# MrGiovanni/R-Super

Hardware: AMD Instinct MI355X
Metric: CT voxels/sec/node (96³ patch, bs=2/GPU) (higher is better)
Workload: dtype bf16; 1 GPU; R-Super 3D UNet(base 32, 26 classes, BasicBlock/IN) full training step (fwd + masked BCE + Dice loss + bwd + clip + AdamW + EMA), 96^3 patches, batch 2/GPU (BASELINE.json configs[1]); global_batch=2, patch=96, parallelism=dp1, sanity_checks_form=device-side flags read one step late (train_ddp.StepGuard)

## Files before the change

include/rsuper_hip.h:

```cpp
#ifndef RSUPER_HIP_H
#define RSUPER_HIP_H
#include <stddef.h>
#include <stdint.h>
#ifdef __cplusplus
extern "C" {
#endif

#define RSUPER_F32 0
#define RSUPER_BF16 1
#define RSUPER_OK 0
#define RSUPER_ERR_ARG 1
#define RSUPER_ERR_LAUNCH 2
#define RSUPER_ERR_UNSUPPORTED 3
#define RSUPER_ERR_NO_DEVICE 4

const char* rsuper_version(void);
int rsuper_device_check(void);


size_t rsuper_conv3_packed_elems(int dtype, int ka, int kb, int n_cols, int bn);

int rsuper_conv3_pack_weights(int dtype, int mode, const float* wa, const float* wb, int ka, int kb, int na, int nb,
                              int bn, void* packed, void* stream);

int rsuper_conv3_pack_weights_batch(int dtype, int n, const int* host_desc, const float* const* host_wa, const float* const* host_wb,
                                    const size_t* host_out_elems, void* packed, void* stream);

int rsuper_conv3_tiles(int D, int H, int W);

int rsuper_conv3_variant(int v);
int rsuper_conv3_wgrad2_min_tiles(int t);

int rsuper_conv3_plan(int dtype, int epi, int N, int D, int H, int W, int Ca, int Cb, int n_cols, int src_flags, int bn, int* plan);

int rsuper_conv3_box_bn(int dtype, int N, int D, int H, int W, int n_cols);

int rsuper_conv3_kd_bn(int dtype, int epi, int N, int D, int H, int W, int n_cols, int src_flags);

int rsuper_conv3_set_workspace(void* ptr, size_t bytes);
size_t rsuper_conv3_workspace_bytes(void);

int rsuper_conv3_part_rows(int dtype, int epi, int N, int D, int H, int W, int n_cols, int bn, int src_flags);

int rsuper_conv3_igemm(int dtype, int epi,
                       const void* xa, int lda, int Ca, const float* mra,
                       const void* xb, int ldb, int Cb, const float* mrb,
                       const void* packed, int n_cols, int bn, int N, int D, int H, int W,
                       void* out, int ldo, const void* res, int ldr, float* part,
                       const void* exa, int elda, int eCa, const float* emra,
                       const void* exb, int eldb, int eCb, const float* emrb, void* stream);
int rsuper_conv3_igemm_split_out(int dtype, int epi,
                                 const void* xa, int lda, int Ca, const float* mra,
                                 const void* xb, int ldb, int Cb, const float* mrb,
                                 const void* packed, int n_cols, int bn, int N, int D, int H, int W,
                                 void* out, int ldo, const void* res, int ldr, float* part,
                                 const void* exa, int elda, int eCa, const float* emra,
                                 const void* exb, int eldb, int eCb, const float* emrb, int out_split, long long out_part, void* stream);
int rsuper_conv3_s2_part_rows(int dtype, int mode, int Ca, int Cb, int n_cols, int N, int FD, int FH, int FW);
int rsuper_conv3_igemm_s2(int dtype, int mode, const void* xa, int lda, int Ca, const float* mra,
                          const void* xb, int ldb, int Cb, const void* packed, int n_cols, int N, int FD, int FH, int FW,
                          void* out, int ldo, float* part, const void* exa, int elda, const float* emra, void* stream);

int rsuper_conv3_wgrad_plan(int dtype, int use_tr, int Ca, int Cb, int Ya, int Yb, int N, int D, int H, int W, int src_flags, int splits, int* plan);
int rsuper_conv3_wgrad_splits(int dtype, int Ca, int Cb, int Ya, int Yb, int N, int D, int H, int W);

int rsuper_conv3_wgrad(int dtype, int use_tr,
                       const void* xa, int lda, int Ca, const float* mra,
                       const void* xb, int ldb, int Cb, const float* mrb,
                       const void* ya, int ldya, int Ya, const void* yb, int ldyb, int Yb,
                       float* dwa, float* dwb, float* workspace, int N, int D, int H, int W, int splits, void* stream);

int rsuper_conv3_wgrad_partial(int dtype, int use_tr, const void* xa, int lda, int Ca, const float* mra,
                               const void* xb, int ldb, int Cb, const float* mrb,
                               const void* ya, int ldya, int Ya, const void* yb, int ldyb, int Yb,
                               float* workspace, int N, int D, int H, int W, int splits, void* stream);
int rsuper_conv3_wgrad_reduce(const float* workspace, int splits, int Cin, int Ya, int Yb, float* dwa, float* dwb, void* stream);
int rsuper_conv3_wgrad_reduce_batch(int n, const void* const* workspaces, const int* splits, const int* Cin, const int* Ya, const int* Yb,
                                    void* const* dwa, void* const* dwb, void* stream);
int rsuper_conv3_wgrad_reduce_batch_stats(int n, const void* const* workspaces, const int* splits, const int* Cin, const int* Ya, const int* Yb,
                                           void* const* dwa, void* const* dwb, int nstats, const void* const* parts, const int* sN, const int* snblk,
                                           const int* sC, const double* scnt, const int* smode, const int* ssplit, void* const* souts, float eps, void* stream);

int rsuper_conv3_wgrad_s2_splits(int dtype, int Ca, int Mtot, int N, int FD, int FH, int FW);
int rsuper_conv3_wgrad_s2(int dtype, const void* xa, int lda, int Ca, const float* mra,
                          const void* ya, int ldya, int Ya, const void* yb, int ldyb, int Yb,
                          float* dwa, float* dwb, float* workspace, int N, int FD, int FH, int FW, int splits, void* stream);

size_t rsuper_pointwise_packed_bytes(int dtype, int K, int N);
int rsuper_pointwise(int dtype, int mode, const float* x, int ldx, const float* w, const float* bias, const float* res, int ldr,
                     float* y, int ldy, long R, int K, int N, void* packed, void* stream);
int rsuper_pointwise_pack_batch(int dtype, const long long* table, int n, long total_items, void* arena, void* stream);
int rsuper_pointwise_wgrad_splits(long R, int N, int K);
int rsuper_pointwise_wgrad(int dtype, const float* dy, int ldy, const float* x, int ldx, long R, int N, int K, float* workspace, int splits,
                           float* dw, float* db, void* stream);

int rsuper_stats_finalize(const float* part, int N, int nblk, int C, double cnt, float eps, int mode, int split, float* out, void* stream);
int rsuper_glue_variant(int v);
int rsuper_in_bwd_finalize(int dtype, const void* g, int ldg, const void* x, int ldx, const float* mr, const float* gm,
                           const void* add1, int lda1, const void* add2, int lda2, void* out, int ldo,
                           int N, int vox, int C, void* stream);

int rsuper_maxpool2_fwd(int dtype, const void* x, int ldx, void* y, int ldy, float* part, int blocks,
                        int N, int D, int H, int W, int C, void* stream);
int rsuper_maxpool2_bwd(int dtype, const void* x, int ldx, const void* dy, int lddy, void* dx, int lddx,
                        int N, int D, int H, int W, int C, void* stream);
int rsuper_maxpool2_bwd_add(int dtype, const void* x, int ldx, const void* dy, int lddy, const void* add, int lda, void* dx, int lddx,
                            int N, int D, int H, int W, int C, void* stream);

int rsuper_subsample2_fwd(int dtype, const void* x, int ldx, void* y, int ldy, float* part, int blocks,
                          int N, int D, int H, int W, int C, void* stream);
int rsuper_subsample2_bwd(int dtype, const void* dy, int lddy, void* dx, int lddx, int N, int D, int H, int W, int C, void* stream);

int rsuper_upsample_fwd(int dtype, const void* x, int ldx, void* y, int ldy, float* part, int blocks,
                        int N, int ID, int IH, int IW, int OD, int OH, int OW, int C, void* stream);
int rsuper_upsample_bwd(int dtype, const void* dy, int lddy, void* dx, int lddx,
                        int N, int ID, int IH, int IW, int OD, int OH, int OW, int C, void* stream);

int rsuper_stem_fwd(int dtype, const float* x, const float* w, void* y, int ldy, float* part,
                    int N, int D, int H, int W, int C, void* stream);
int rsuper_stem_wgrad(int dtype, const float* x, const void* dy, int lddy, float* dw, int N, int D, int H, int W, int C, void* stream);

int rsuper_head_fwd(int dtype, const void* x, int ldx, const float* w, const float* b, float* logits, int N, int vox, int C, int K, void* stream);
int rsuper_head_bwd_data(int dtype, const float* dlogits, const float* w, void* dx, int lddx, int N, int vox, int C, int K, void* stream);
int rsuper_head_bwd_weight(int dtype, const void* x, int ldx, const float* dlogits, float* dw, float* db, int N, int vox, int C, int K, void* stream);
int rsuper_head_bwd(int dtype, const void* x, int ldx, const float* dlogits, const float* w, void* dx, int lddx, float* dw, float* db,
                    int N, int vox, int C, int K, void* stream);

int rsuper_plane_partials_fwd(const float* x, size_t xstride, const uint8_t* t, const uint8_t* k, const float* w1, const uint8_t* w2,
                              double* sums, int flags, int planes, size_t V, void* stream);
int rsuper_plane_partials_bwd(const float* x, size_t xstride, const uint8_t* t, const uint8_t* k, const float* w1, const uint8_t* w2,
                              const float* g, float* dx, int flags, int planes, size_t V, void* stream);
int rsuper_plane_partials_fwd2(const float* x, size_t xstride, const uint8_t* t, const uint8_t* tpk, int tP, int tC, const uint8_t* k, const uint8_t* kflags,
                               const float* w1, const uint8_t* w2, double* sums, int flags, int planes, size_t V, void* stream);
int rsuper_plane_partials_bwd2(const float* x, size_t xstride, const uint8_t* t, const uint8_t* tpk, int tP, int tC, const uint8_t* k, const uint8_t* kflags,
                               const float* w1, const uint8_t* w2, const float* g, float* dx, int flags, int planes, size_t V, void* stream);
int rsuper_plane_partials_blocks(size_t V);
int rsuper_plane_partials_fwd3(const float* x, size_t xstride, const uint8_t* t, const uint8_t* tpk, int tP, int tC, const uint8_t* k, const uint8_t* kflags,
                               const float* w1, const uint8_t* w2, double* pblk, int flags, int planes, size_t V, void* stream);
int rsuper_plane_sums_reduce(const double* pblk, int rows, int nb, float* out, void* stream);
int rsuper_seg_from_sums(const float* sums, const float* cw, int B, int C, size_t V, double scale, float* loss, float* dsums, void* stream);
int rsuper_report_from_sums(const float* sums, const float* roww, int R, int B, int L, size_t V, int use_vol, const float* flags, const float* rvol,
                            double tol, double E, int nplans, const int* plan, int apply_dice, int standard_ce, float* loss, float* jac, void* stream);
int rsuper_sigmoid_mask(const float* x, const uint8_t* m, float* out, size_t V, void* stream);

int rsuper_window_accumulate(const float* logits, float* acc, int BK, int wd, int wh, int ww, int D, int H, int W, int d0, int h0, int w0,
                             int assign, void* stream);
int rsuper_window_normalize(float* acc, const float* cd, const float* ch, const float* cw, long BK, int D, int H, int W, void* stream);

int rsuper_cnorm_rows(long vox);
int rsuper_cnorm_small(const float* x, const float* dy, const float* mr, float* out, float* mr_out, int N, long vox, int C, int relu, float eps,
                       int mode, void* stream);
int rsuper_cnorm_stats(const float* x, const float* dy, const float* mr, float* part, int N, long vox, int C, int relu, int mode, void* stream);
int rsuper_cnorm_forward(const float* x, float* part, float* mr, float* y, int N, long vox, int C, int relu, float eps, void* stream);
int rsuper_cnorm_backward(const float* x, const float* dy, const float* mr, float* part, float* gm, float* dx, int N, long vox, int C, int relu,
                          void* stream);
int rsuper_cnorm_apply(const float* x, const float* dy, const float* mr, const float* gm, float* out, int N, long vox, int C, int relu, int mode,
                       void* stream);

int rsuper_se_forward(const float* x, const float* w1, const float* b1, const float* w2, const float* b2, float* part, float* ms, float* tab,
                      float* hbuf, float* y, int N, long vox, int C, int r, void* stream);
int rsuper_se_backward(const float* x, const float* dy, const float* ident, const float* w1, const float* w2, const float* ms, const float* tab,
                       const float* hbuf, float* part, float* gm, float* dz1, float* tab2, float* dx, float* dw1, float* db1, float* dw2, float* db2,
                       int N, long vox, int C, int r, void* stream);

int rsuper_cl_planar(const float* src, float* dst, int N, long vox, int C, int K, int to_channels_last, void* stream);

int rsuper_token_attn_supported(int L, int dim_head);
int rsuper_token_attn_fwd(const float* qkv, float* o, float* p, int B, int L, int heads, int dim_head, float scale, void* stream);
int rsuper_token_attn_bwd(const float* qkv, const float* o, const float* p, const float* d_o, float* d_qkv, int B, int L, int heads, int dim_head, float scale,
                          void* stream);

int rsuper_battn_supported(int T, int dim_head, int heads);
int rsuper_battn_chunks(int L, int heads);
int rsuper_battn_fwd(const float* fqv, const float* mqv, float* f_out, float* m_out, float* lse, float* part, float* pms, int B, int L, int T,
                     int heads, int dim_head, float scale, void* stream);
int rsuper_battn_bwd(const float* fqv, const float* mqv, const float* m_out, const float* lse, const float* d_f_out, const float* d_m_out,
                     float* d_fqv, float* d_mqv, float* part, int B, int L, int T, int heads, int dim_head, float scale, void* stream);

int rsuper_depthwise3_rows(long vox);
int rsuper_depthwise3_fwd(const float* x, const float* w, float* y, int N, int D, int H, int W, int C, int flip, void* stream);
int rsuper_depthwise3_wgrad(const float* x, const float* dy, float* part, float* dw, int N, int D, int H, int W, int C, void* stream);

int rsuper_dilate_volume(const uint8_t* in, uint8_t* out, uint8_t* tmp, long nvol, int D, int H, int W, int kernel_size, void* stream);
int rsuper_dilate_volume_sparse(const uint8_t* in, uint8_t* out, uint8_t* tmp, const uint8_t* flags, long nvol, int D, int H, int W,
                                int kernel_size, void* stream);
long rsuper_ball_workspace_floats(int D, int H, int W, int d_odd);
int rsuper_ball_conv_argmax(const float* x, int D, int H, int W, int d_odd, float std, unsigned long long* best, float* conv_out, float* workspace,
                            void* stream);
int rsuper_insert_ball(uint8_t* out, int D, int H, int W, int cz, int cy, int cx, int d_odd, int half, unsigned int* count, void* stream);
int rsuper_insert_ball_at(uint8_t* out, int D, int H, int W, const unsigned long long* best, int d_odd, int half, unsigned int* count, void* stream);
int rsuper_radix_hist(const float* x, const uint8_t* m, long V, uint32_t prefix, int shift, unsigned int* hist256, void* stream);
int rsuper_topk_mark(const float* x, const uint8_t* m, long V, uint32_t thr_bits, unsigned int need_eq, uint8_t* out, void* stream);
int rsuper_topk_select(const float* x, const uint8_t* m, long V, unsigned int k, uint8_t* out, unsigned int* workspace, void* stream);
int rsuper_topk_select_multi(const float* x, const uint8_t* m, long V, const unsigned int* k, int nk, uint8_t* out, unsigned int* workspace,
                             int clip_to_mask, void* stream);
int rsuper_compact(const float* x, const uint8_t* pm, long V, float* vals, uint32_t* idx, unsigned int* n, void* stream);
int rsuper_rank_weights(const float* vals, const uint32_t* idx, unsigned int n, float log2_d, float scale, float* w, void* stream);
int rsuper_rank_assign(const long long* ids, unsigned int n, float log2_d, float scale, float* w, void* stream);
int rsuper_plane_any(const uint8_t* m, long planes, long V, uint8_t* flags, void* stream);
// ... 132 lines not shown
```

r-super_amd/csrc/api.hip:

```cpp
#include <string.h>
#include <math.h>
#include <stdlib.h>
#include "common.hpp"
#include "kernels.hpp"
#include "misc.hpp"
#include "loss.hpp"
#include "morph.hpp"
#include "optim.hpp"
#include "../../include/rsuper_hip.h"

#define ST(s) ((hipStream_t)(s))

static inline bool dt_ok(int dt) { return dt == RS_F32 || dt == RS_BF16; }
static inline bool ch_ok(int C, int ld) { return C >= 0 && (C % 8) == 0 && (ld % 8) == 0 && ld >= C; }
static inline bool bn_ok(int bn) { return bn == 32 || bn == 64 || bn == 96 || bn == 128; }
static inline int ntiles_for(int n_cols, int bn) { const int per = bn / 32; return ((n_cols + bn - 1) / bn) * per; }
static inline int pack_cols(int mode, int na, int nb) { return mode == 1 ? (nb ? (nb & 0xFFFF) : na) : na + nb; }
static inline bool pack_range_ok(int mode, int na, int nb) { return mode != 1 || nb == 0 || ((nb >> 16) % 32 == 0 && (nb & 0xFFFF) > 0 && (nb >> 16) + (nb & 0xFFFF) <= na); }

#include "igemm_plan.hpp"
#include "wgrad_plan.hpp"

template <typename F>
static int for_chunks(int n, void* const* p, void* const* g, void* const* m, void* const* v, void* const* e, const size_t* numel, F f) {
    for (int i0 = 0; i0 < n; i0 += RS_MT_MAX) {
        MTChunk c;
        memset(&c, 0, sizeof(c));
        c.n = n - i0 < RS_MT_MAX ? n - i0 : RS_MT_MAX;
        int blk = 0;
        for (int i = 0; i < c.n; ++i) {
            c.p[i] = p ? p[i0 + i] : nullptr; c.g[i] = g ? g[i0 + i] : nullptr; c.m[i] = m ? m[i0 + i] : nullptr;
            c.v[i] = v ? v[i0 + i] : nullptr; c.ema[i] = e ? e[i0 + i] : nullptr;
            c.numel[i] = numel[i0 + i];
            c.blk_start[i] = blk;
            blk += rs_mt_blocks(numel[i0 + i]);
        }
        c.blk_start[c.n] = blk;
        if (blk == 0) continue;
        const int rc = f(c);
        if (rc) return rc;
    }
    return RS_OK;
}


extern "C" {

const char* rsuper_version(void) { return "rsuper-hip 0.1 (gfx950)"; }

int rsuper_device_check(void) {
    int n = 0;
    if (hipGetDeviceCount(&n) != hipSuccess || n < 1) return RSUPER_ERR_NO_DEVICE;
    int dev = 0;
    if (hipGetDevice(&dev) != hipSuccess) return RSUPER_ERR_NO_DEVICE;
    hipDeviceProp_t p;
    if (hipGetDeviceProperties(&p, dev) != hipSuccess) return RSUPER_ERR_NO_DEVICE;
    return strncmp(p.gcnArchName, "gfx950", 6) == 0 ? RSUPER_OK : RSUPER_ERR_NO_DEVICE;
}

size_t rsuper_conv3_packed_elems(int dtype, int ka, int kb, int n_cols, int bn) {
    if (!dt_ok(dtype) || !bn_ok(bn)) return 0;
    return rs_packed_elems(dtype, ka, kb, ntiles_for(n_cols, bn));
}

int rsuper_conv3_pack_weights(int dtype, int mode, const float* wa, const float* wb, int ka, int kb, int na, int nb,
                              int bn, void* packed, void* stream) {
    if (!dt_ok(dtype) || !wa || !packed || (mode != 0 && mode != 1) || ka <= 0 || kb < 0 || na <= 0 || nb < 0) return RS_ERR_ARG;
    if ((kb > 0 || nb > 0) && mode == 1 && kb > 0 && !wb) return RS_ERR_ARG;
    if (mode == 0 && nb > 0 && !wb) return RS_ERR_ARG;
    if (!bn_ok(bn)) return RS_ERR_ARG;
    PackParams q;
    q.wa = wa; q.wb = wb; q.mode = mode; q.ka = ka; q.kb = kb; q.na = na; q.nb = nb;
    if (!pack_range_ok(mode, na, nb)) return RS_ERR_ARG;
    q.ntiles = ntiles_for(pack_cols(mode, na, nb), bn);
    return rs_launch_pack(q, dtype, packed, ST(stream));
}

int rsuper_conv3_pack_weights_batch(int dtype, int n, const int* host_desc, const float* const* host_wa, const float* const* host_wb,
                                    const size_t* host_out_elems, void* packed, void* stream) {
    if (!dt_ok(dtype) || n <= 0 || !host_desc || !host_wa || !host_wb || !host_out_elems || !packed) return RS_ERR_ARG;
    const int KP = dtype == RS_F32 ? 4 : 8;
    for (int i0 = 0; i0 < n; i0 += RS_PACK_BATCH_MAX) {
        PackBatch b;
        memset(&b, 0, sizeof(b));
        b.n = n - i0 < RS_PACK_BATCH_MAX ? n - i0 : RS_PACK_BATCH_MAX;
        const size_t base = host_out_elems[i0];
        for (int i = 0; i < b.n; ++i) {
            const int* d = host_desc + (size_t)(i0 + i) * 6;
            if ((d[0] != 0 && d[0] != 1) || d[1] <= 0 || d[2] < 0 || d[3] <= 0 || d[4] < 0 || !bn_ok(d[5])) return RS_ERR_ARG;
            PackParams& q = b.q[i];
            q.wa = host_wa[i0 + i]; q.wb = host_wb[i0 + i]; q.mode = d[0]; q.ka = d[1]; q.kb = d[2]; q.na = d[3]; q.nb = d[4];
            if (!pack_range_ok(d[0], d[3], d[4])) return RS_ERR_ARG;
            q.ntiles = ntiles_for(pack_cols(d[0], d[3], d[4]), d[5]);
            if (!q.wa || ((host_out_elems[i0 + i] - base) % KP)) return RS_ERR_ARG;
            b.vec_start[i] = (host_out_elems[i0 + i] - base) / KP;
        }
        const int* dl = host_desc + (size_t)(i0 + b.n - 1) * 6;
        b.vec_start[b.n] = b.vec_start[b.n - 1] + rs_packed_elems(dtype, dl[1], dl[2], ntiles_for(pack_cols(dl[0], dl[3], dl[4]), dl[5])) / KP;
        for (int i = 0; i + 1 < b.n; ++i) {
            const int* d = host_desc + (size_t)(i0 + i) * 6;
            if (b.vec_start[i] + rs_packed_elems(dtype, d[1], d[2], ntiles_for(pack_cols(d[0], d[3], d[4]), d[5])) / KP != b.vec_start[i + 1]) return RS_ERR_ARG;
        }
        const int rc = rs_launch_pack_batch(b, dtype, (char*)packed + base * (dtype == RS_F32 ? 4 : 2), ST(stream));
        if (rc) return rc;
// ... 235 lines not shown
}

int rsuper_conv3_wgrad_s2_splits(int dtype, int Ca, int Mtot, int N, int FD, int FH, int FW) {
    if (!dt_ok(dtype) || Ca <= 0 || Mtot <= 0 || N <= 0 || FD <= 0 || FH <= 0 || FW <= 0) return -1;
    return rs_wgrad_s2_splits(dtype, Ca, Mtot, N, FD, FH, FW);
}
int rsuper_conv3_wgrad_s2(int dtype, const void* xa, int lda, int Ca, const float* mra,
                          const void* ya, int ldya, int Ya, const void* yb, int ldyb, int Yb,
                          float* dwa, float* dwb, float* workspace, int N, int FD, int FH, int FW, int splits, void* stream) {
    if (!dt_ok(dtype) || !xa || !ya || !dwa || !workspace || !ch_ok(Ca, lda) || Ca == 0 || !ch_ok(Ya, ldya) || Ya == 0) return RS_ERR_ARG;
    if (Yb > 0 && (!yb || !dwb || !ch_ok(Yb, ldyb))) return RS_ERR_ARG;
    if (N <= 0 || FD <= 0 || FH <= 0 || FW <= 0 || splits <= 0) return RS_ERR_ARG;
    if ((unsigned long long)N * FD * FH * FW * (unsigned long long)lda * (dtype == RS_F32 ? 4 : 2) >= (1ull << 32)) return RS_ERR_UNSUPPORTED;
    WgradParams p;
    memset(&p, 0, sizeof(p));
    p.xa = {xa, lda, Ca, mra};
    p.ya = {ya, ldya, Ya, nullptr};
    p.yb = {yb, ldyb, Yb > 0 ? Yb : 0, nullptr};
    p.dwa = dwa; p.dwb = dwb; p.ws = workspace; p.N = N; p.D = FD; p.H = FH; p.W = FW; p.splits = splits;
    return rs_launch_wgrad_s2(p, dtype, ST(stream));
}

size_t rsuper_pointwise_packed_bytes(int dtype, int K, int N) { return dt_ok(dtype) && K > 0 && N > 0 ? rs_pw_packed_bytes(N, K, dtype) : 0; }
int rsuper_pointwise(int dtype, int mode, const float* x, int ldx, const float* w, const float* bias, const float* res, int ldr,
                     float* y, int ldy, long R, int K, int N, void* packed, void* stream) {
    if (!dt_ok(dtype) || (mode != 0 && mode != 1) || !x || !y || !packed || R <= 0 || K <= 0 || N <= 0) return RS_ERR_ARG;
    if ((N % 4) || (ldx % 4) || (ldy % 4) || ldx < K || ldy < N || (mode == 1 && bias)) return RS_ERR_ARG;
    if (res && ((ldr % 4) || ldr < N)) return RS_ERR_ARG;
    if ((unsigned long long)R * ldx * 4ull >= (1ull << 32) || R > 0x7FFFFFFFl) return RS_ERR_UNSUPPORTED;
    return rs_launch_pointwise(dtype, mode, x, ldx, w, bias, res, ldr, y, ldy, (int)R, K, N, packed, ST(stream));
}

int rsuper_pointwise_pack_batch(int dtype, const long long* table, int n, long total_items, void* arena, void* stream) {
    if (!dt_ok(dtype) || !table || n <= 0 || total_items <= 0 || !arena) return RS_ERR_ARG;
    return rs_launch_pointwise_pack_batch(dtype, table, n, total_items, arena, ST(stream));
}
int rsuper_pointwise_wgrad_splits(long R, int N, int K) { return (R > 0 && R <= 0x7FFFFFFFl && N > 0 && K > 0) ? rs_pw_wgrad_splits((int)R, N, K) : 0; }
int rsuper_pointwise_wgrad(int dtype, const float* dy, int ldy, const float* x, int ldx, long R, int N, int K, float* workspace, int splits,
                           float* dw, float* db, void* stream) {
    if (!dt_ok(dtype) || !dy || !x || !workspace || !dw || R <= 0 || N <= 0 || K <= 0 || splits <= 0) return RS_ERR_ARG;
    if ((N % 4) || (K % 4) || ldy < N || ldx < K) return RS_ERR_ARG;
    if ((unsigned long long)(R + 1) * ldx * 4ull >= (1ull << 32) || (unsigned long long)(R + 1) * ldy * 4ull >= (1ull << 32)) return RS_ERR_UNSUPPORTED;
    return rs_launch_pointwise_wgrad(dtype, dy, ldy, x, ldx, (int)R, N, K, workspace, splits, dw, db, ST(stream));
}

int rsuper_stats_finalize(const float* part, int N, int nblk, int C, double cnt, float eps, int mode, int split, float* out, void* stream) {
    if (!part || !out || N <= 0 || nblk <= 0 || C <= 0 || cnt <= 0 || split < 0 || split >= C || (mode != 0 && mode != 1)) return RS_ERR_ARG;
    return rs_launch_stats_finalize(part, N, nblk, C, cnt, eps, mode, split, out, ST(stream));
}

int rsuper_glue_variant(int v) { return rs_glue_variant(v); }

int rsuper_in_bwd_finalize(int dtype, const void* g, int ldg, const void* x, int ldx, const float* mr, const float* gm,
                           const void* add1, int lda1, const void* add2, int lda2, void* out, int ldo,
                           int N, int vox, int C, void* stream) {
    if (!dt_ok(dtype) || !g || !x || !mr || !gm || !out || !ch_ok(C, ldg) || !ch_ok(C, ldx) || !ch_ok(C, ldo)) return RS_ERR_ARG;
    InBwdParams p = {g, ldg, x, ldx, mr, gm, add1, lda1, add2, lda2, out, ldo, N, vox, C};
    return rs_launch_in_bwd(p, dtype, ST(stream));
}

int rsuper_maxpool2_fwd(int dtype, const void* x, int ldx, void* y, int ldy, float* part, int blocks,
                        int N, int D, int H, int W, int C, void* stream) {
    if (!dt_ok(dtype) || !x || !y || !ch_ok(C, ldx) || !ch_ok(C, ldy) || blocks <= 0 || D < 2 || H < 2 || W < 2) return RS_ERR_ARG;
    PoolParams p = {x, ldx, y, ldy, nullptr, 0, part, N, D, H, W, C};
    return rs_launch_pool(p, dtype, 0, blocks, ST(stream));
}
int rsuper_maxpool2_bwd(int dtype, const void* x, int ldx, const void* dy, int lddy, void* dx, int lddx,
                        int N, int D, int H, int W, int C, void* stream) {
    if (!dt_ok(dtype) || !x || !dy || !dx || !ch_ok(C, ldx) || !ch_ok(C, lddy) || !ch_ok(C, lddx)) return RS_ERR_ARG;
    if ((D & 1) || (H & 1) || (W & 1)) {
        if (lddx != C) return RS_ERR_UNSUPPORTED;
        if (const int rc = rs_launch_zero_bytes(dx, (size_t)N * D * H * W * C * (dtype == RS_F32 ? 4 : 2), ST(stream))) return rc;
    }
    PoolParams p = {x, ldx, (void*)dy, lddy, dx, lddx, nullptr, N, D, H, W, C};
    return rs_launch_pool(p, dtype, 1, 1, ST(stream));
}
int rsuper_maxpool2_bwd_add(int dtype, const void* x, int ldx, const void* dy, int lddy, const void* add, int lda, void* dx, int lddx,
                            int N, int D, int H, int W, int C, void* stream) {
    if (!dt_ok(dtype) || !x || !dy || !add || !dx || !ch_ok(C, ldx) || !ch_ok(C, lddy) || !ch_ok(C, lda) || !ch_ok(C, lddx)) return RS_ERR_ARG;
    if ((D & 1) || (H & 1) || (W & 1)) return RS_ERR_UNSUPPORTED;
    PoolParams p = {x, ldx, (void*)dy, lddy, dx, lddx, nullptr, N, D, H, W, C, add, lda};
    return rs_launch_pool(p, dtype, 1, 1, ST(stream));
}

int rsuper_subsample2_fwd(int dtype, const void* x, int ldx, void* y, int ldy, float* part, int blocks,
                          int N, int D, int H, int W, int C, void* stream) {
    if (!dt_ok(dtype) || !x || !y || !ch_ok(C, ldx) || !ch_ok(C, ldy) || blocks <= 0 || D < 1 || H < 1 || W < 1 || N <= 0) return RS_ERR_ARG;
    PoolParams p = {x, ldx, y, ldy, nullptr, 0, part, N, D, H, W, C};
    return rs_launch_subsample(p, dtype, 0, blocks, ST(stream));
}
int rsuper_subsample2_bwd(int dtype, const void* dy, int lddy, void* dx, int lddx, int N, int D, int H, int W, int C, void* stream) {
    if (!dt_ok(dtype) || !dy || !dx || !ch_ok(C, lddy) || !ch_ok(C, lddx) || D < 1 || H < 1 || W < 1 || N <= 0) return RS_ERR_ARG;
    PoolParams p = {nullptr, 0, (void*)dy, lddy, dx, lddx, nullptr, N, D, H, W, C};
    return rs_launch_subsample(p, dtype, 1, 1, ST(stream));
}

int rsuper_upsample_fwd(int dtype, const void* x, int ldx, void* y, int ldy, float* part, int blocks,
                        int N, int ID, int IH, int IW, int OD, int OH, int OW, int C, void* stream) {
    if (!dt_ok(dtype) || !x || !y || !ch_ok(C, ldx) || !ch_ok(C, ldy) || blocks <= 0) return RS_ERR_ARG;
    UpParams p = {x, ldx, y, ldy, nullptr, 0, part, N, ID, IH, IW, OD, OH, OW, C};
    return rs_launch_upsample(p, dtype, 0, blocks, ST(stream));
}
int rsuper_upsample_bwd(int dtype, const void* dy, int lddy, void* dx, int lddx,
                        int N, int ID, int IH, int IW, int OD, int OH, int OW, int C, void* stream) {
    if (!dt_ok(dtype) || !dy || !dx || !ch_ok(C, lddy) || !ch_ok(C, lddx)) return RS_ERR_ARG;
    UpParams p = {nullptr, 0, (void*)dy, lddy, dx, lddx, nullptr, N, ID, IH, IW, OD, OH, OW, C};
    return rs_launch_upsample(p, dtype, 1, 1, ST(stream));
}
int rsuper_stem_fwd(int dtype, const float* x, const float* w, void* y, int ldy, float* part,
                    int N, int D, int H, int W, int C, void* stream) {
    if (!dt_ok(dtype) || !x || !w || !y || !part || !ch_ok(C, ldy)) return RS_ERR_ARG;
    StemParams p = {x, w, y, ldy, part, nullptr, N, D, H, W, C};
    return rs_launch_stem(p, dtype, 0, ST(stream));
}
int rsuper_stem_wgrad(int dtype, const float* x, const void* dy, int lddy, float* dw, int N, int D, int H, int W, int C, void* stream) {
    if (!dt_ok(dtype) || !x || !dy || !dw || !ch_ok(C, lddy)) return RS_ERR_ARG;
    StemParams p = {x, nullptr, (void*)dy, lddy, nullptr, dw, N, D, H, W, C};
    return rs_launch_stem(p, dtype, 1, ST(stream));
}

int rsuper_head_fwd(int dtype, const void* x, int ldx, const float* w, const float* b, float* logits, int N, int vox, int C, int K, void* stream) {
    if (!dt_ok(dtype) || !x || !w || !b || !logits || !ch_ok(C, ldx) || K <= 0) return RS_ERR_ARG;
    HeadParams p = {x, ldx, w, b, logits, nullptr, 0, nullptr, nullptr, N, vox, C, K};
    return rs_launch_head(p, dtype, 0, ST(stream));
}
int rsuper_head_bwd_data(int dtype, const float* dlogits, const float* w, void* dx, int lddx, int N, int vox, int C, int K, void* stream) {
    if (!dt_ok(dtype) || !dlogits || !w || !dx || !ch_ok(C, lddx) || K <= 0) return RS_ERR_ARG;
    HeadParams p = {nullptr, 0, w, nullptr, (float*)dlogits, dx, lddx, nullptr, nullptr, N, vox, C, K};
    return rs_launch_head(p, dtype, 1, ST(stream));
}
int rsuper_head_bwd_weight(int dtype, const void* x, int ldx, const float* dlogits, float* dw, float* db, int N, int vox, int C, int K, void* stream) {
    if (!dt_ok(dtype) || !x || !dlogits || !dw || !db || !ch_ok(C, ldx) || K <= 0) return RS_ERR_ARG;
    HeadParams p = {x, ldx, nullptr, nullptr, (float*)dlogits, nullptr, 0, dw, db, N, vox, C, K};
    return rs_launch_head(p, dtype, 2, ST(stream));
}

int rsuper_head_bwd(int dtype, const void* x, int ldx, const float* dlogits, const float* w, void* dx, int lddx, float* dw, float* db,
                    int N, int vox, int C, int K, void* stream) {
    if (!dt_ok(dtype) || !x || !dlogits || !w || !dx || !dw || !db || !ch_ok(C, ldx) || !ch_ok(C, lddx) || K <= 0) return RS_ERR_ARG;
    if (dtype == RS_BF16 && K <= 32 && C <= 32) {
        HeadParams p = {x, ldx, w, nullptr, (float*)dlogits, dx, lddx, dw, db, N, vox, C, K};
        return rs_launch_head(p, dtype, 2, ST(stream));
    }
    const int rc = rsuper_head_bwd_data(dtype, dlogits, w, dx, lddx, N, vox, C, K, stream);
    return rc ? rc : rsuper_head_bwd_weight(dtype, x, ldx, dlogits, dw, db, N, vox, C, K, stream);
}

int rsuper_plane_partials_fwd(const float* x, size_t xstride, const uint8_t* t, const uint8_t* k, const float* w1, const uint8_t* w2,
                              double* sums, int flags, int planes, size_t V, void* stream) {
    if (!x || !sums || planes <= 0 || V == 0 || (flags & ~2)) return RS_ERR_ARG;
    PlaneParams p = {x, xstride, t, k, w1, w2, sums, nullptr, nullptr, 0, V, k ? (flags >> 1) & 1 : 0, nullptr, 0, 0, nullptr};
    return rs_launch_plane_partials(p, planes, 0, ST(stream));
}
int rsuper_plane_partials_fwd2(const float* x, size_t xstride, const uint8_t* t, const uint8_t* tpk, int tP, int tC, const uint8_t* k, const uint8_t* kflags,
                               const float* w1, const uint8_t* w2, double* sums, int flags, int planes, size_t V, void* stream) {
    if (!x || !sums || planes <= 0 || V == 0 || (flags & ~2) || (t && tpk)) return RS_ERR_ARG;
    if (tpk && (tC <= 0 || tP * 8 < tC || planes % tC)) return RS_ERR_ARG;
    PlaneParams p = {x, xstride, t, k, w1, w2, sums, nullptr, nullptr, 0, V, k ? (flags >> 1) & 1 : 0, tpk, tP, tC, kflags, nullptr};
    return rs_launch_plane_partials(p, planes, 0, ST(stream));
}
int rsuper_plane_partials_blocks(size_t V) { return V ? rs_plane_partials_blocks(V) : 0; }
int rsuper_plane_partials_fwd3(const float* x, size_t xstride, const uint8_t* t, const uint8_t* tpk, int tP, int tC, const uint8_t* k, const uint8_t* kflags,
                               const float* w1, const uint8_t* w2, double* pblk, int flags, int planes, size_t V, void* stream) {
    if (!x || !pblk || planes <= 0 || V == 0 || (flags & ~2) || (t && tpk)) return RS_ERR_ARG;
    if (tpk && (tC <= 0 || tP * 8 < tC || planes % tC)) return RS_ERR_ARG;
    PlaneParams p = {x, xstride, t, k, w1, w2, nullptr, nullptr, nullptr, 0, V, k ? (flags >> 1) & 1 : 0, tpk, tP, tC, kflags, pblk};
    return rs_launch_plane_partials(p, planes, 0, ST(stream));
}
int rsuper_plane_sums_reduce(const double* pblk, int rows, int nb, float* out, void* stream) {
    if (!pblk || !out || rows <= 0 || nb <= 0) return RS_ERR_ARG;
    return rs_launch_plane_sums_reduce(pblk, rows, nb, out, ST(stream));
}
int rsuper_plane_partials_bwd(const float* x, size_t xstride, const uint8_t* t, const uint8_t* k, const float* w1, const uint8_t* w2,
                              const float* g, float* dx, int flags, int planes, size_t V, void* stream) {
    if (!x || !g || !dx || planes <= 0 || V == 0 || (flags & ~3)) return RS_ERR_ARG;
    PlaneParams p = {x, xstride, t, k, w1, w2, nullptr, g, dx, flags & 1, V, k ? (flags >> 1) & 1 : 0, nullptr, 0, 0, nullptr, nullptr};
    return rs_launch_plane_partials(p, planes, 1, ST(stream));
}
int rsuper_plane_partials_bwd2(const float* x, size_t xstride, const uint8_t* t, const uint8_t* tpk, int tP, int tC, const uint8_t* k, const uint8_t* kflags,
                               const float* w1, const uint8_t* w2, const float* g, float* dx, int flags, int planes, size_t V, void* stream) {
    if (!x || !g || !dx || planes <= 0 || V == 0 || (flags & ~3) || (t && tpk)) return RS_ERR_ARG;
    if (tpk && (tC <= 0 || tP * 8 < tC || planes % tC)) return RS_ERR_ARG;
    PlaneParams p = {x, xstride, t, k, w1, w2, nullptr, g, dx, flags & 1, V, k ? (flags >> 1) & 1 : 0, tpk, tP, tC, kflags};
    return rs_launch_plane_partials(p, planes, 1, ST(stream));
}
int rsuper_cnorm_rows(long vox) { return rs_cnorm_rows(vox); }
int rsuper_cnorm_stats(const float* x, const float* dy, const float* mr, float* part, int N, long vox, int C, int relu, int mode, void* stream) {
    if (!x || !part || N <= 0 || vox <= 0 || C <= 0 || (C & 3) || (mode != 0 && mode != 1) || (mode == 1 && (!dy || !mr))) return RS_ERR_ARG;
    return rs_launch_cnorm_stats(x, dy, mr, part, N, vox, C, relu ? 1 : 0, mode, ST(stream));
}
// ... 275 lines not shown
```

r-super_amd/csrc/misc.hpp:

```cpp
#pragma once
#include <hip/hip_runtime.h>
#include <stddef.h>
#include <stdint.h>

struct InBwdParams {
    const void* g; int ldg;
    const void* x; int ldx;
    const float* mr;
    const float* gm;
    const void* add1; int lda1;
    const void* add2; int lda2;
    void* out; int ldo;
    int N, vox, C;
};

struct PoolParams {
    const void* x; int ldx;
    void* y; int ldy;
    void* dx; int lddx;
    float* part;
    int N, D, H, W, C;
    const void* add; int lda;
};

struct UpParams {
    const void* x; int ldx;
    void* y; int ldy;
    void* dx; int lddx;
    float* part;
    int N, ID, IH, IW, OD, OH, OW, C;
};

struct StemParams {
    const float* x;
    const float* w;
    void* y; int ldy;
    float* part;
    float* dw;
    int N, D, H, W, C;
};

struct HeadParams {
    const void* x; int ldx;
    const float* w; const float* b;
    float* logits;
    void* dx; int lddx;
    float* dw; float* db;
    int N, vox, C, K;
};

int rs_cnorm_rows(long vox);
int rs_launch_cnorm_small(const float* x, const float* dy, const float* mr, float* out, float* mr_out, int N, long vox, int C, int relu, float eps, int mode, hipStream_t st);
int rs_launch_cnorm_stats(const float* x, const float* dy, const float* mr, float* part, int N, long vox, int C, int relu, int mode, hipStream_t st);
int rs_launch_cnorm_apply(const float* x, const float* dy, const float* mr, const float* gm, float* out, int N, long vox, int C, int relu, int mode, hipStream_t st);
int rs_battn_supported(int T, int dh, int heads);
int rs_battn_chunks(int L, int heads);
int rs_launch_battn(const float* fqv, const float* mqv, float* fout, float* mout, float* lse, const float* dfo, const float* dmo,
                    float* dfqv, float* dmqv, float* part, float* pms, int B, int L, int T, int heads, int dh, float scale, int bwd,
                    hipStream_t st);
int rs_launch_se_forward(const float* x, const float* w1, const float* b1, const float* w2, const float* b2, float* part, float* ms, float* tab,
                         float* hbuf, float* y, int N, long vox, int C, int r, hipStream_t st);
int rs_launch_se_backward(const float* x, const float* dy, const float* ident, const float* w1, const float* w2, const float* ms, const float* tab,
                          const float* hbuf, float* part, float* gm, float* dz1buf, float* tab2, float* dx, float* dw1, float* db1, float* dw2,
                          float* db2, int N, long vox, int C, int r, hipStream_t st);
int rs_launch_cl_planar(const float* src, float* dst, int N, long vox, int C, int K, int dir, hipStream_t st);
int rs_depthwise_rows(long vox);
int rs_launch_depthwise(const float* x, const float* w, float* y, int N, int D, int H, int W, int C, int flip, hipStream_t st);
int rs_launch_depthwise_wgrad(const float* x, const float* dy, float* part, float* dw, int N, int D, int H, int W, int C, hipStream_t st);
int rs_launch_stats_finalize(const float* part, int N, int nblk, int C, double cnt, float eps, int mode, int split, float* out, hipStream_t st);
int rs_elem_blocks(size_t items);
int rs_glue_variant(int v);
int rs_launch_in_bwd(const InBwdParams& p, int dtype, hipStream_t st);
int rs_launch_pool(const PoolParams& p, int dtype, int bwd, int blocks, hipStream_t st);
int rs_launch_subsample(const PoolParams& p, int dtype, int bwd, int blocks, hipStream_t st);
int rs_launch_upsample(const UpParams& p, int dtype, int bwd, int blocks, hipStream_t st);
int rs_launch_stem(const StemParams& p, int dtype, int wgrad, hipStream_t st);
int rs_launch_head(const HeadParams& p, int dtype, int which, hipStream_t st);
```

r-super_amd/csrc/unet_misc.hip:

```cpp
#include <string.h>
#include "common.hpp"
#include "kernels.hpp"
#include "misc.hpp"

namespace {

__global__ __launch_bounds__(1024) void stats_finalize_kernel(const float* part, int nblk, int C, double cnt, float eps, int mode, int split, float* out) {
    __shared__ double red[32][32][2];
    const int n = blockIdx.y;
    const int cl = threadIdx.x & 31, g = threadIdx.x >> 5;
    const int c = blockIdx.x * 32 + cl;
    double s0 = 0.0, s1 = 0.0;
    if (c < C) {
        const float* base = part + ((size_t)n * nblk * C + c) * 2;
        int b = g;
        for (; b + 96 < nblk; b += 128) {
            const float2 v0 = *(const float2*)(base + (size_t)b * C * 2), v1 = *(const float2*)(base + (size_t)(b + 32) * C * 2);
            const float2 v2 = *(const float2*)(base + (size_t)(b + 64) * C * 2), v3 = *(const float2*)(base + (size_t)(b + 96) * C * 2);
            s0 += ((double)v0.x + (double)v1.x) + ((double)v2.x + (double)v3.x);
            s1 += ((double)v0.y + (double)v1.y) + ((double)v2.y + (double)v3.y);
        }
        for (; b < nblk; b += 32) {
            const float2 v = *(const float2*)(base + (size_t)b * C * 2);
            s0 += (double)v.x; s1 += (double)v.y;
        }
    }
    red[g][cl][0] = s0; red[g][cl][1] = s1;
    __syncthreads();
    if (g == 0 && c < C) {
        for (int k = 1; k < 32; ++k) { s0 += red[k][cl][0]; s1 += red[k][cl][1]; }
        float* o = split <= 0 ? out + ((size_t)n * C + c) * 2
                   : c < split ? out + ((size_t)n * split + c) * 2
                               : out + (size_t)gridDim.y * split * 2 + ((size_t)n * (C - split) + (c - split)) * 2;
        if (mode == 0) {
            const double mean = s0 / cnt;
            double var = s1 / cnt - mean * mean;
            if (var < 0.0) var = 0.0;
            o[0] = (float)mean;
            o[1] = (float)(1.0 / sqrt(var + (double)eps));
        } else {
            o[0] = (float)(s0 / cnt); o[1] = (float)(s1 / cnt);
        }
    }
}

template <int KP>
__device__ __forceinline__ void block_channel_sums(const float* s1, const float* s2, int C, int CV, int VL, int vl, int s,
                                                   bool active, float* part_blk) {
    extern __shared__ __attribute__((aligned(16))) char smem[];
    float* red = (float*)smem;
    if (active) {
#pragma unroll
        for (int j = 0; j < KP; ++j) {
            red[((vl * C) + s * KP + j) * 2] = s1[j];
            red[((vl * C) + s * KP + j) * 2 + 1] = s2[j];
        }
    }
    __syncthreads();
    for (int c = threadIdx.x; c < C; c += blockDim.x) {
        float a = 0.f, b = 0.f;
        for (int v = 0; v < VL; ++v) { a += red[(v * C + c) * 2]; b += red[(v * C + c) * 2 + 1]; }
        part_blk[c * 2] = a; part_blk[c * 2 + 1] = b;
    }
}

template <typename T>
__global__ __launch_bounds__(256) void in_bwd_finalize_kernel(InBwdParams p) {
    constexpr int KP = Elem<T>::KP;
    const uint32_t CV = (uint32_t)p.C / KP;
    const uint32_t total = (uint32_t)p.vox * CV;
    const uint32_t n = blockIdx.y;
    const uint32_t stride = gridDim.x * 256u;
    const bool fixed_slot = (256u % CV) == 0;
    const T* gp = (const T*)p.g + (size_t)n * p.vox * p.ldg;
    const T* xp = (const T*)p.x + (size_t)n * p.vox * p.ldx;
    const T* a1p = p.add1 ? (const T*)p.add1 + (size_t)n * p.vox * p.lda1 : nullptr;
    const T* a2p = p.add2 ? (const T*)p.add2 + (size_t)n * p.vox * p.lda2 : nullptr;
    T* op = (T*)p.out + (size_t)n * p.vox * p.ldo;
    float mu[KP], rs[KP], m1[KP], m2[KP];
    auto constants = [&](uint32_t c) {
#pragma unroll
        for (int j = 0; j < KP; ++j) {
            const size_t o = ((size_t)n * p.C + c + j) * 2;
            mu[j] = p.mr[o]; rs[j] = p.mr[o + 1]; m1[j] = p.gm[o]; m2[j] = p.gm[o + 1];
        }
    };
    uint32_t i = blockIdx.x * 256u + threadIdx.x;
    uint32_t v = i / CV, c = (i - v * CV) * KP;
    const uint32_t vstep = stride / CV;
    if (fixed_slot && i < total) constants(c);
    for (; i < total; i += stride, v += vstep) {
        if (!fixed_slot) { v = i / CV; c = (i - v * CV) * KP; constants(c); }
        float g[KP], x[KP], o[KP];
        const uint4 gq = *(const uint4*)(gp + (size_t)v * p.ldg + c);
        const uint4 xq = *(const uint4*)(xp + (size_t)v * p.ldx + c);
        uint4 a1q = make_uint4(0, 0, 0, 0), a2q = make_uint4(0, 0, 0, 0);
        if (a1p) a1q = *(const uint4*)(a1p + (size_t)v * p.lda1 + c);
        if (a2p) a2q = *(const uint4*)(a2p + (size_t)v * p.lda2 + c);
        unpack16<T>(gq, g);
        unpack16<T>(xq, x);
#pragma unroll
        for (int j = 0; j < KP; ++j) {
            const float xn = (x[j] - mu[j]) * rs[j];
            o[j] = rs[j] * (g[j] - m1[j] - xn * m2[j]);
        }
        if (a1p) {
            float a[KP];
            unpack16<T>(a1q, a);
#pragma unroll
            for (int j = 0; j < KP; ++j) o[j] += a[j];
        }
        if (a2p) {
            float a[KP];
            unpack16<T>(a2q, a);
#pragma unroll
            for (int j = 0; j < KP; ++j) o[j] += a[j];
        }
        *(uint4*)(op + (size_t)v * p.ldo + c) = pack16<T>(o);
    }
}

template <typename T, int U>
__global__ __launch_bounds__(256) void in_bwd_finalize2_kernel(InBwdParams p, int cv_shift) {
    constexpr int KP = Elem<T>::KP;
    const uint32_t CV = 1u << cv_shift;
    const uint32_t total = (uint32_t)p.vox * CV;
    const uint32_t n = blockIdx.y;
    const uint32_t i0 = blockIdx.x * (256u * U) + threadIdx.x;
    if (i0 >= total) return;
    const T* gp = (const T*)p.g + (size_t)n * p.vox * p.ldg;
    const T* xp = (const T*)p.x + (size_t)n * p.vox * p.ldx;
    const T* a1p = p.add1 ? (const T*)p.add1 + (size_t)n * p.vox * p.lda1 : nullptr;
    const T* a2p = p.add2 ? (const T*)p.add2 + (size_t)n * p.vox * p.lda2 : nullptr;
    T* op = (T*)p.out + (size_t)n * p.vox * p.ldo;
    const uint32_t c = (i0 & (CV - 1u)) * KP;
    uint4 gq[U], xq[U], a1q[U], a2q[U];
#pragma unroll
    for (int u = 0; u < U; ++u) {
        const uint32_t i = i0 + 256u * u;
        const uint32_t v = (i < total ? i : i0) >> cv_shift;
        gq[u] = *(const uint4*)(gp + (size_t)v * p.ldg + c);
        xq[u] = *(const uint4*)(xp + (size_t)v * p.ldx + c);
        a1q[u] = make_uint4(0, 0, 0, 0); a2q[u] = make_uint4(0, 0, 0, 0);
        if (a1p) a1q[u] = *(const uint4*)(a1p + (size_t)v * p.lda1 + c);
        if (a2p) a2q[u] = *(const uint4*)(a2p + (size_t)v * p.lda2 + c);
    }
    float mu[KP], rs[KP], m1[KP], m2[KP];
#pragma unroll
    for (int j = 0; j < KP; ++j) {
        const size_t o = ((size_t)n * p.C + c + j) * 2;
        mu[j] = p.mr[o]; rs[j] = p.mr[o + 1]; m1[j] = p.gm[o]; m2[j] = p.gm[o + 1];
    }
#pragma unroll
    for (int u = 0; u < U; ++u) {
        const uint32_t i = i0 + 256u * u;
        if (i >= total) break;
        const uint32_t v = i >> cv_shift;
        float g[KP], x[KP], o[KP];
        unpack16<T>(gq[u], g);
        unpack16<T>(xq[u], x);
#pragma unroll
        for (int j = 0; j < KP; ++j) {
            const float xn = (x[j] - mu[j]) * rs[j];
            o[j] = rs[j] * (g[j] - m1[j] - xn * m2[j]);
        }
        if (a1p) {
            float a[KP];
            unpack16<T>(a1q[u], a);
#pragma unroll
            for (int j = 0; j < KP; ++j) o[j] += a[j];
        }
        if (a2p) {
            float a[KP];
            unpack16<T>(a2q[u], a);
#pragma unroll
            for (int j = 0; j < KP; ++j) o[j] += a[j];
        }
        *(uint4*)(op + (size_t)v * p.ldo + c) = pack16<T>(o);
    }
}

template <typename T>
__global__ void maxpool_fwd_kernel(PoolParams p) {
    constexpr int KP = Elem<T>::KP;
    const int CV = p.C / KP, VL = 256 / CV;
    const int vl = threadIdx.x / CV, s = threadIdx.x % CV;
    const bool active = vl < VL;
    const int n = blockIdx.y;
    const int OD = p.D / 2, OH = p.H / 2, OW = p.W / 2;
    const int ovox = OD * OH * OW;
    const int per_blk = (ovox + gridDim.x - 1) / gridDim.x;
    const int v0 = blockIdx.x * per_blk, v1 = min(ovox, v0 + per_blk);
    float s1[KP], s2[KP];
#pragma unroll
    for (int j = 0; j < KP; ++j) { s1[j] = 0.f; s2[j] = 0.f; }
    if (active)
        for (int v = v0 + vl; v < v1; v += VL) {
            const int ow = v % OW, oh = (v / OW) % OH, od = v / (OW * OH);
            float m[KP];
#pragma unroll
            for (int j = 0; j < KP; ++j) m[j] = -INFINITY;
#pragma unroll
            for (int k = 0; k < 8; ++k) {
                const int d = od * 2 + (k >> 2), h = oh * 2 + ((k >> 1) & 1), w = ow * 2 + (k & 1);
                float x[KP];
                unpack16<T>(*(const uint4*)((const T*)p.x + ((((size_t)n * p.D + d) * p.H + h) * p.W + w) * (size_t)p.ldx + s * KP), x);
#pragma unroll
                for (int j = 0; j < KP; ++j) m[j] = fmaxf(m[j], x[j]);
            }
            *(uint4*)((T*)p.y + ((size_t)n * ovox + v) * p.ldy + s * KP) = pack16<T>(m);
#pragma unroll
            for (int j = 0; j < KP; ++j) { s1[j] += m[j]; s2[j] += m[j] * m[j]; }
        }
    if (p.part) block_channel_sums<KP>(s1, s2, p.C, CV, VL, vl, s, active, p.part + ((size_t)n * gridDim.x + blockIdx.x) * p.C * 2);
}

template <typename T, int U>
__global__ __launch_bounds__(256) void maxpool_fwd2_kernel(PoolParams p) {
    constexpr int KP = Elem<T>::KP;
    const int CV = p.C / KP, VL = 256 / CV;
    const int CVb = CV / gridDim.z;
    const int vl = threadIdx.x / CVb, s = blockIdx.z * CVb + threadIdx.x % CVb;
    const bool active = vl < VL;
    const int n = blockIdx.y;
    const int OD = p.D / 2, OH = p.H / 2, OW = p.W / 2;
    const int ovox = OD * OH * OW;
    const int per_blk = (ovox + gridDim.x - 1) / gridDim.x;
    const int v0 = blockIdx.x * per_blk, v1 = min(ovox, v0 + per_blk);
    float s1[KP], s2[KP];
#pragma unroll
    for (int j = 0; j < KP; ++j) { s1[j] = 0.f; s2[j] = 0.f; }
    if (active)
        for (int v = v0 + vl; v < v1; v += U * VL) {
            uint4 q[U][8];
#pragma unroll
            for (int u = 0; u < U; ++u) {
                const int vv = v + u * VL < v1 ? v + u * VL : v;
                const int ow = vv % OW, oh = (vv / OW) % OH, od = vv / (OW * OH);
#pragma unroll
                for (int k = 0; k < 8; ++k) {
                    const int d = od * 2 + (k >> 2), h = oh * 2 + ((k >> 1) & 1), w = ow * 2 + (k & 1);
                    q[u][k] = *(const uint4*)((const T*)p.x + ((((size_t)n * p.D + d) * p.H + h) * p.W + w) * (size_t)p.ldx + s * KP);
                }
            }
#pragma unroll
            for (int u = 0; u < U; ++u) {
                if (v + u * VL >= v1) break;
                float m[KP];
#pragma unroll
                for (int j = 0; j < KP; ++j) m[j] = -INFINITY;
#pragma unroll
                for (int k = 0; k < 8; ++k) {
                    float x[KP];
                    unpack16<T>(q[u][k], x);
#pragma unroll
                    for (int j = 0; j < KP; ++j) m[j] = fmaxf(m[j], x[j]);
                }
                *(uint4*)((T*)p.y + ((size_t)n * ovox + v + u * VL) * p.ldy + s * KP) = pack16<T>(m);
#pragma unroll
                for (int j = 0; j < KP; ++j) { s1[j] += m[j]; s2[j] = fmaf(m[j], m[j], s2[j]); }
            }
        }
    const int Cb = CVb * KP;
    if (p.part)
        block_channel_sums<KP>(s1, s2, Cb, CVb, VL, vl, threadIdx.x % CVb, active,
                               p.part + (((size_t)n * gridDim.x + blockIdx.x) * p.C + (size_t)blockIdx.z * Cb) * 2);
}

template <typename T>
__global__ void maxpool_bwd_kernel(PoolParams p) {
    constexpr int KP = Elem<T>::KP;
    const int CV = p.C / KP;
    const int n = blockIdx.y;
    const int OD = p.D / 2, OH = p.H / 2, OW = p.W / 2;
    const size_t total = (size_t)OD * OH * OW * CV;
    for (size_t i = (size_t)blockIdx.x * blockDim.x + threadIdx.x; i < total; i += (size_t)gridDim.x * blockDim.x) {
        const int s = (int)(i % CV); const int v = (int)(i / CV);
        const int ow = v % OW, oh = (v / OW) % OH, od = v / (OW * OH);
        float x[8][KP], m[KP], dy[KP];
#pragma unroll
        for (int j = 0; j < KP; ++j) m[j] = -INFINITY;
#pragma unroll
        for (int k = 0; k < 8; ++k) {
            const int d = od * 2 + (k >> 2), h = oh * 2 + ((k >> 1) & 1), w = ow * 2 + (k & 1);
            unpack16<T>(*(const uint4*)((const T*)p.x + ((((size_t)n * p.D + d) * p.H + h) * p.W + w) * (size_t)p.ldx + s * KP), x[k]);
#pragma unroll
            for (int j = 0; j < KP; ++j) m[j] = fmaxf(m[j], x[k][j]);
        }
        unpack16<T>(*(const uint4*)((const T*)p.y + ((size_t)n * OD * OH * OW + v) * p.ldy + s * KP), dy);
        bool done[KP];
#pragma unroll
        for (int j = 0; j < KP; ++j) done[j] = false;
#pragma unroll
        for (int k = 0; k < 8; ++k) {
            const int d = od * 2 + (k >> 2), h = oh * 2 + ((k >> 1) & 1), w = ow * 2 + (k & 1);
            float o[KP];
#pragma unroll
            for (int j = 0; j < KP; ++j) {
                const bool hit = !done[j] && x[k][j] == m[j];
                o[j] = hit ? dy[j] : 0.f;
                done[j] = done[j] || hit;
            }
            if (p.add) {
                float a[KP];
                unpack16<T>(*(const uint4*)((const T*)p.add + ((((size_t)n * p.D + d) * p.H + h) * p.W + w) * (size_t)p.lda + s * KP), a);
#pragma unroll
                for (int j = 0; j < KP; ++j) o[j] += a[j];
            }
            *(uint4*)((T*)p.dx + ((((size_t)n * p.D + d) * p.H + h) * p.W + w) * (size_t)p.lddx + s * KP) = pack16<T>(o);
        }
    }
}

template <typename T>
__global__ void subsample_fwd_kernel(PoolParams p) {
    constexpr int KP = Elem<T>::KP;
    const int CV = p.C / KP, VL = 256 / CV;
    const int CVb = CV / gridDim.z;
    const int vl = threadIdx.x / CVb, s = blockIdx.z * CVb + threadIdx.x % CVb;
    const bool active = vl < VL;
    const int n = blockIdx.y;
    const int OD = (p.D + 1) / 2, OH = (p.H + 1) / 2, OW = (p.W + 1) / 2;
    const int ovox = OD * OH * OW;
    const int per_blk = (ovox + gridDim.x - 1) / gridDim.x;
    const int v0 = blockIdx.x * per_blk, v1 = min(ovox, v0 + per_blk);
    float s1[KP], s2[KP];
#pragma unroll
    for (int j = 0; j < KP; ++j) { s1[j] = 0.f; s2[j] = 0.f; }
    if (active)
        for (int v = v0 + vl; v < v1; v += VL) {
            const int ow = v % OW, oh = (v / OW) % OH, od = v / (OW * OH);
            const uint4 q = *(const uint4*)((const T*)p.x + ((((size_t)n * p.D + 2 * od) * p.H + 2 * oh) * p.W + 2 * ow) * (size_t)p.ldx + s * KP);
            *(uint4*)((T*)p.y + ((size_t)n * ovox + v) * p.ldy + s * KP) = q;
            float m[KP];
            unpack16<T>(q, m);
#pragma unroll
            for (int j = 0; j < KP; ++j) { s1[j] += m[j]; s2[j] += m[j] * m[j]; }
        }
    const int Cb = CVb * KP;
    if (p.part)
        block_channel_sums<KP>(s1, s2, Cb, CVb, VL, vl, threadIdx.x % CVb, active,
                               p.part + (((size_t)n * gridDim.x + blockIdx.x) * p.C + (size_t)blockIdx.z * Cb) * 2);
}

template <typename T>
__global__ void subsample_bwd_kernel(PoolParams p) {
    constexpr int KP = Elem<T>::KP;
    const int CV = p.C / KP;
    const int n = blockIdx.y;
    const int OH = (p.H + 1) / 2, OW = (p.W + 1) / 2, OD = (p.D + 1) / 2;
    const size_t total = (size_t)p.D * p.H * p.W * CV;
    for (size_t i = (size_t)blockIdx.x * blockDim.x + threadIdx.x; i < total; i += (size_t)gridDim.x * blockDim.x) {
        const int s = (int)(i % CV); const size_t v = i / CV;
        const int w = (int)(v % p.W), h = (int)((v / p.W) % p.H), d = (int)(v / ((size_t)p.W * p.H));
        uint4 q = make_uint4(0, 0, 0, 0);
        if (!((d | h | w) & 1))
            q = *(const uint4*)((const T*)p.y + (((size_t)n * OD + d / 2) * OH + h / 2) * OW * (size_t)p.ldy + (size_t)(w / 2) * p.ldy + s * KP);
        *(uint4*)((T*)p.dx + ((size_t)n * p.D * p.H * p.W + v) * (size_t)p.lddx + s * KP) = q;
    }
}

__host__ __device__ __forceinline__ void lin_coord(int o, float scale, int I, int& i0, int& i1, float& l1) {
#pragma clang fp contract(off)
    const float src = scale * (float)o;
    i0 = (int)src;
    if (i0 > I - 1) i0 = I - 1;
    i1 = i0 + (i0 < I - 1 ? 1 : 0);
    l1 = src - (float)i0;
}

template <typename T>
__global__ void upsample_fwd_kernel(UpParams p) {
    constexpr int KP = Elem<T>::KP;
    const int CV = p.C / KP, VL = 256 / CV;
    const int vl = threadIdx.x / CV, s = threadIdx.x % CV;
    const bool active = vl < VL;
    const int n = blockIdx.y;
    const int ovox = p.OD * p.OH * p.OW;
    const int per_blk = (ovox + gridDim.x - 1) / gridDim.x;
    const int v0 = blockIdx.x * per_blk, v1 = min(ovox, v0 + per_blk);
    const float sd = p.OD > 1 ? (float)(p.ID - 1) / (float)(p.OD - 1) : 0.f;
    const float sh = p.OH > 1 ? (float)(p.IH - 1) / (float)(p.OH - 1) : 0.f;
    const float sw = p.OW > 1 ? (float)(p.IW - 1) / (float)(p.OW - 1) : 0.f;
    float s1[KP], s2[KP];
#pragma unroll
    for (int j = 0; j < KP; ++j) { s1[j] = 0.f; s2[j] = 0.f; }
    if (active)
        for (int v = v0 + vl; v < v1; v += 2 * VL) {
// ... 297 lines not shown
#pragma unroll
        for (int c = 0; c < NW; ++c) wc[c] = c < nc ? ew->w[c] : 0.f;
        float acc[KP];
#pragma unroll
        for (int j = 0; j < KP; ++j) acc[j] = 0.f;
        for (int a = 0; a < na; ++a) {
            const float wa = ed->w[a];
            for (int b = 0; b < nb; ++b) {
                const float wdh = wa * eh->w[b];
                const uint32_t rowo = ((uint32_t)(ed->lo + a) * (uint32_t)p.OH + (uint32_t)(eh->lo + b)) * (uint32_t)p.OW + (uint32_t)wlo;
                uint4 q[NW];
#pragma unroll
                for (int c = 0; c < NW; ++c) {
                    const uint32_t off = c < nc ? ((rowo + c) * (uint32_t)p.ldy + s * KP) * (uint32_t)sizeof(T) : 0xFFFFFFFFu;
                    const auto r = __builtin_amdgcn_raw_buffer_load_b128(rs, off, 0, 0);
                    q[c] = make_uint4(r[0], r[1], r[2], r[3]);
                }
#pragma unroll
                for (int c = 0; c < NW; ++c) {
                    float g[KP];
                    unpack16<T>(q[c], g);
                    const float wt = wdh * wc[c];
#pragma unroll
                    for (int j = 0; j < KP; ++j) acc[j] = fmaf(wt, g[j], acc[j]);
                }
            }
        }
        *(uint4*)((T*)p.dx + ((size_t)n * p.ID * p.IH * p.IW + v) * p.lddx + s * KP) = pack16<T>(acc);
    }
}

template <typename T>
__global__ __launch_bounds__(256) void upsample_bwd2_kernel(UpParams p) {
    extern __shared__ __attribute__((aligned(16))) char smem[];
    UpEnt* tab = (UpEnt*)smem;
    __shared__ int nwmax;
    if (threadIdx.x == 0) nwmax = 0;
    __syncthreads();
    const float sd = p.OD > 1 ? (float)(p.ID - 1) / (float)(p.OD - 1) : 0.f;
    const float sh = p.OH > 1 ? (float)(p.IH - 1) / (float)(p.OH - 1) : 0.f;
    const float sw = p.OW > 1 ? (float)(p.IW - 1) / (float)(p.OW - 1) : 0.f;
    for (int t = threadIdx.x; t < p.ID + p.IH + p.IW; t += 256) {
        const int axis = t < p.ID ? 0 : (t < p.ID + p.IH ? 1 : 2);
        const int i = axis == 0 ? t : (axis == 1 ? t - p.ID : t - p.ID - p.IH);
        const float sc = axis == 0 ? sd : (axis == 1 ? sh : sw);
        const int I = axis == 0 ? p.ID : (axis == 1 ? p.IH : p.IW), O = axis == 0 ? p.OD : (axis == 1 ? p.OH : p.OW);
        int lo, hi;
        up_range(i, sc, O, lo, hi);
        constexpr int CAND = 16;
        float cw[CAND];
        int first = CAND, last = -1;
#pragma unroll
        for (int k = 0; k < CAND; ++k) {
            cw[k] = lo + k <= hi ? up_weight(lo + k, i, sc, I) : 0.f;
            if (cw[k] != 0.f) { if (first == CAND) first = k; last = k; }
        }
        UpEnt e;
        e.lo = lo + (first == CAND ? 0 : first);
        e.n = last < 0 ? 0 : min(last - first + 1, UP_MAXW);
#pragma unroll
        for (int k = 0; k < UP_MAXW; ++k) {
            float wv = 0.f;
#pragma unroll
            for (int m = 0; m < CAND; ++m) if (m == first + k && m <= last) wv = cw[m];
            e.w[k] = wv;
        }
        tab[t] = e;
        if (axis == 2) atomicMax(&nwmax, e.n);
    }
    __syncthreads();
    const UpEnt* td = tab; const UpEnt* th = tab + p.ID; const UpEnt* tw = tab + p.ID + p.IH;
    const uint32_t CV = (uint32_t)p.C / Elem<T>::KP;
    const uint32_t total = (uint32_t)(p.ID * p.IH * p.IW) * CV;
    const uint32_t i0 = blockIdx.x * 256u + threadIdx.x, stride = gridDim.x * 256u;
    if (nwmax <= 4) up_bwd_rows<T, 4>(p, td, th, tw, blockIdx.y, i0, total, stride);
    else if (nwmax <= 6) up_bwd_rows<T, 6>(p, td, th, tw, blockIdx.y, i0, total, stride);
    else up_bwd_rows<T, UP_MAXW>(p, td, th, tw, blockIdx.y, i0, total, stride);
}

struct UpInParams {
    const void* g; int ldg;
    void* dx; int lddx;
    int N, ID, IH, IW, OD, OH, OW, C;
};
#ifndef UP4_SL
#define UP4_SL 2
#endif
constexpr int UP4_ROWS = 16;
template <int NT>
__global__ __launch_bounds__(256, 3) void upsample_bwd4_kernel(UpInParams p, int nbx) {
    typedef bf16_t T;
    constexpr int CPT = 8, NWD = CPT / 2;
    constexpr int SL = UP4_SL;
    __shared__ float Wd[UP4_ROWS][2], Wh[UP4_ROWS][2];
    __shared__ float4 W4[UP4_ROWS * UP4_ROWS];
    __shared__ int span[4];
    const int tid = threadIdx.x, n = blockIdx.y;
    const int CV = p.C / CPT, tiles_h = (p.IH + 1) / 2;
    int L;
    {
        const int nt = gridDim.x, b = blockIdx.x;
        const int q = nt >> 3, r = nt & 7, xcd = b & 7, k = b >> 3;
        L = (xcd < r ? xcd * (q + 1) : r * (q + 1) + (xcd - r) * q) + k;
    }
    const int bx = L % nbx, tile = L / nbx;
    const int id0 = (tile / tiles_h) * 2, ih0 = (tile % tiles_h) * 2;
    const float sd = p.OD > 1 ? (float)(p.ID - 1) / (float)(p.OD - 1) : 0.f;
    const float sh = p.OH > 1 ? (float)(p.IH - 1) / (float)(p.OH - 1) : 0.f;
    const float sw = p.OW > 1 ? (float)(p.IW - 1) / (float)(p.OW - 1) : 0.f;
    if (tid < 128) {
        const int axis = tid >> 6, r = tid & 63;
        const int i0 = axis ? ih0 : id0, I = axis ? p.IH : p.ID, O = axis ? p.OH : p.OD;
        const float sc = axis ? sh : sd;
        int lo, hi, lo2, hi2;
        up_range(i0, sc, O, lo, hi);
        if (i0 + 1 < I) { up_range(i0 + 1, sc, O, lo2, hi2); if (hi2 > hi) hi = hi2; }
        const int o = lo + r;
        float w0 = 0.f, w1 = 0.f;
        if (r < UP4_ROWS && o <= hi) { w0 = up_weight(o, i0, sc, I); if (i0 + 1 < I) w1 = up_weight(o, i0 + 1, sc, I); }
        const unsigned long long nz = __ballot(w0 != 0.f || w1 != 0.f);
        const int first = nz ? __builtin_ctzll(nz) : 0, last = nz ? 63 - __builtin_clzll(nz) : -1;
        if (hi - lo + 1 > UP4_ROWS) __builtin_trap();
        if (r >= first && r <= last) { float (*Wt)[2] = axis ? Wh : Wd; Wt[r - first][0] = w0; Wt[r - first][1] = w1; }
        if (r == 0) { span[axis * 2] = lo + first; span[axis * 2 + 1] = last - first + 1; }
    }
    __syncthreads();
    const int od0 = span[0], rd = span[1], oh0 = span[2], rh = span[3];
    const int nrow = rd * rh;
    if (tid < nrow) { const int a = tid / rh, b = tid - a * rh; W4[tid] = make_float4(Wd[a][0] * Wh[b][0], Wd[a][0] * Wh[b][1], Wd[a][1] * Wh[b][0], Wd[a][1] * Wh[b][1]); }
    __syncthreads();
    const int flat = bx * 256 + tid;
    if (flat >= p.IW * CV) return;
    const int iw = flat / CV, s = flat - iw * CV;
    int wlo;
    float wc[NT];
    {
        int lo, hi;
        up_range(iw, sw, p.OW, lo, hi);
        int first = -1;
#pragma unroll
        for (int k = 0; k < 8; ++k)
            if (first < 0 && lo + k <= hi && up_weight(lo + k, iw, sw, p.IW) != 0.f) first = k;
        wlo = lo + (first < 0 ? 0 : first);
#pragma unroll
        for (int c = 0; c < NT; ++c) wc[c] = (first >= 0 && wlo + c <= hi) ? up_weight(wlo + c, iw, sw, p.IW) : 0.f;
        if (first >= 0 && wlo + NT <= hi && up_weight(wlo + NT, iw, sw, p.IW) != 0.f) __builtin_trap();
    }
    const uint32_t ovox = (uint32_t)(p.OD * p.OH * p.OW);
    const uint32_t grow = (uint32_t)p.ldg * 2u;
    const __amdgpu_buffer_rsrc_t grs = __builtin_amdgcn_make_buffer_rsrc((void*)((const T*)p.g + (size_t)n * ovox * p.ldg), 0, ovox * grow, 0x00020000);
    uint32_t goff[NT];
#pragma unroll
    for (int c = 0; c < NT; ++c) {
        const uint32_t v = (uint32_t)(wlo + (wc[c] != 0.f ? c : 0));
        goff[c] = v * grow + (uint32_t)s * 16u;
    }
    float acc[4][CPT];
#pragma unroll
    for (int i = 0; i < 4; ++i)
#pragma unroll
        for (int k = 0; k < CPT; ++k) acc[i][k] = 0.f;
    uint4 gq[SL][NT];
    int ia = 0, ib = 0;
    auto issue = [&](int slot) {
        const uint32_t row = (uint32_t)__builtin_amdgcn_readfirstlane(((od0 + ia) * p.OH + (oh0 + ib)) * p.OW);
#pragma unroll
        for (int c = 0; c < NT; ++c) {
            const auto q = __builtin_amdgcn_raw_buffer_load_b128(grs, goff[c], row * grow, 0);
            gq[slot][c] = make_uint4(q[0], q[1], q[2], q[3]);
        }
        if (++ib == rh) { ib = 0; ++ia; }
    };
#pragma unroll
    for (int h = 0; h < SL - 1; ++h) if (h < nrow) issue(h);
    for (int r = 0; r < nrow; r += SL) {
#pragma unroll
        for (int h = 0; h < SL; ++h) {
            const int rr = r + h;
            if (rr >= nrow) break;
            if (rr + SL - 1 < nrow) issue((h + SL - 1) % SL);
            f32x2_t tg[NWD];
#pragma unroll
            for (int j = 0; j < NWD; ++j) tg[j] = f32x2_t{0.f, 0.f};
#pragma unroll
            for (int c = 0; c < NT; ++c) {
                const f32x2_t w2 = {wc[c], wc[c]};
                const uint32_t wq[4] = {gq[h][c].x, gq[h][c].y, gq[h][c].z, gq[h][c].w};
#pragma unroll
                for (int j = 0; j < NWD; ++j) {
                    const f32x2_t v2 = {__uint_as_float(wq[j] << 16), __uint_as_float(wq[j] & 0xffff0000u)};
                    tg[j] = __builtin_elementwise_fma(w2, v2, tg[j]);
                }
            }
            float t[CPT];
#pragma unroll
            for (int j = 0; j < NWD; ++j) { t[2 * j] = tg[j][0]; t[2 * j + 1] = tg[j][1]; }
            const float4 w4 = W4[rr];
            const float wv[4] = {w4.x, w4.y, w4.z, w4.w};
#pragma unroll
            for (int i = 0; i < 4; ++i)
#pragma unroll
                for (int k = 0; k < CPT; ++k) acc[i][k] = fmaf(wv[i], t[k], acc[i][k]);
        }
    }
#pragma unroll
    for (int i = 0; i < 4; ++i) {
        const int id = id0 + (i >> 1), ih = ih0 + (i & 1);
        if (id < p.ID && ih < p.IH)
            *(uint4*)((T*)p.dx + ((size_t)((n * p.ID + id) * p.IH + ih) * p.IW + iw) * p.lddx + s * CPT) = pack16<T>(acc[i]);
    }
}
static int up_max_count(int I, int O) {
    const float sc = O > 1 ? (float)(I - 1) / (float)(O - 1) : 0.f;
    int m = 1;
    for (int i = 0; i < I; ++i) {
        int lo, hi;
        up_range(i, sc, O, lo, hi);
        int first = -1, last = -2;
        for (int o = lo; o <= hi; ++o)
            if (up_weight(o, i, sc, I) != 0.f) { if (first < 0) first = o; last = o; }
        if (last - first + 1 > m) m = last - first + 1;
    }
    return m;
}
static int up_pair_window(int I, int O) {
    const float sc = O > 1 ? (float)(I - 1) / (float)(O - 1) : 0.f;
    int m = 1;
    for (int i = 0; i < I; i += 2) {
        int lo, hi, lo2, hi2;
        up_range(i, sc, O, lo, hi);
        if (i + 1 < I) { up_range(i + 1, sc, O, lo2, hi2); if (hi2 > hi) hi = hi2; }
        if (hi - lo + 1 > m) m = hi - lo + 1;
    }
    return m;
}

template <typename T, int C>
__global__ __launch_bounds__(256) void stem_fwd_kernel(StemParams p) {
    extern __shared__ __attribute__((aligned(16))) char smem[];
    float* tile = (float*)smem;
    const float* __restrict__ w = p.w;
    const int n = blockIdx.y;
    const int vox = p.D * p.H * p.W;
    const int v = blockIdx.x * 256 + threadIdx.x;
    const bool ok = v < vox;
    float xv[27];
    {
        const int x0 = v % p.W, y0 = (v / p.W) % p.H, z0 = v / (p.W * p.H);
        const float* xin = p.x + (size_t)n * vox;
#pragma unroll
        for (int tap = 0; tap < 27; ++tap) {
            const int z = z0 + tap / 9 - 1, y = y0 + (tap % 9) / 3 - 1, x = x0 + tap % 3 - 1;
            xv[tap] = (ok && z >= 0 && z < p.D && y >= 0 && y < p.H && x >= 0 && x < p.W) ? xin[((size_t)z * p.H + y) * p.W + x] : 0.f;
        }
    }
    constexpr int KP = Elem<T>::KP;
    T* o = (T*)p.y + ((size_t)n * vox + (ok ? v : 0)) * p.ldy;
#pragma unroll 1
    for (int c8 = 0; c8 < C; c8 += KP) {
        float acc[KP];
#pragma unroll
        for (int j = 0; j < KP; ++j) {
            float a = 0.f;
#pragma unroll
            for (int tap = 0; tap < 27; ++tap) a += xv[tap] * w[(c8 + j) * 27 + tap];
            acc[j] = Elem<T>::rnd(a);
            tile[threadIdx.x * (C + 1) + c8 + j] = ok ? acc[j] : 0.f;
        }
        if (ok) *(uint4*)(o + c8) = pack16<T>(acc);
    }
// ... 344 lines not shown
    for (int k = 0; k < p.K; ++k) {
        const float g = p.logits[((size_t)n * p.K + k) * p.vox + v];
#pragma unroll
        for (int c = 0; c < C; ++c) f[c] += g * w[k * C + c];
    }
    T* dx = (T*)p.dx + ((size_t)n * p.vox + v) * p.lddx;
#pragma unroll
    for (int c = 0; c < C; c += KP) *(uint4*)(dx + c) = pack16<T>(f + c);
}

template <typename F> void set_smem(F k, size_t smem) {
    if (smem > 64 * 1024) (void)hipFuncSetAttribute((const void*)k, hipFuncAttributeMaxDynamicSharedMemorySize, (int)smem);
}

}

int rs_launch_stats_finalize(const float* part, int N, int nblk, int C, double cnt, float eps, int mode, int split, float* out, hipStream_t st) {
    hipLaunchKernelGGL(stats_finalize_kernel, dim3((C + 31) / 32, N), dim3(1024), 0, st, part, nblk, C, cnt, eps, mode, split, out);
    return rs_check_launch();
}

int rs_elem_blocks(size_t items) {
    size_t b = (items + 255) / 256;
    return (int)(b < 1 ? 1 : (b > 4096 ? 4096 : b));
}

int rs_glue_variant(int v) {
    static int g = !(getenv("RSUPER_GLUE_KERNELS") && atoi(getenv("RSUPER_GLUE_KERNELS")) == 0);
    if (v == 0 || v == 1) g = v;
    return g;
}

static int stat_csplit(int rows, int N, int CV) {
    if (!rs_glue_variant(-1)) return 1;
    const int VL = 256 / CV;
    int z = 1;
    while ((size_t)rows * N * z < 1024 && CV % (2 * z) == 0 && CV / (2 * z) >= 8 && (CV / (2 * z)) * VL >= 64) z *= 2;
    return z;
}

int rs_launch_in_bwd(const InBwdParams& p, int dtype, hipStream_t st) {
    const int KP = dtype == RS_F32 ? 4 : 8;
    if ((size_t)p.vox * (p.C / KP) >= 0xFFFFFFFFull) return RS_ERR_UNSUPPORTED;
    const int blocks = rs_elem_blocks((size_t)p.vox * (p.C / KP));
    const uint32_t CV = (uint32_t)(p.C / KP);
    const size_t nb1 = ((size_t)p.vox * CV + 255) / 256;
    if (rs_glue_variant(-1) && CV > 0 && (CV & (CV - 1)) == 0 && CV <= 256 && nb1 >= 256 && nb1 <= 8192) {
        const int sh = __builtin_ctz(CV);
        if (nb1 >= 1024) {
            const dim3 grid((unsigned)((nb1 + 3) / 4), p.N);
            if (dtype == RS_F32) hipLaunchKernelGGL((in_bwd_finalize2_kernel<float, 4>), grid, dim3(256), 0, st, p, sh);
            else hipLaunchKernelGGL((in_bwd_finalize2_kernel<bf16_t, 4>), grid, dim3(256), 0, st, p, sh);
        } else {
            const dim3 grid((unsigned)((nb1 + 1) / 2), p.N);
            if (dtype == RS_F32) hipLaunchKernelGGL((in_bwd_finalize2_kernel<float, 2>), grid, dim3(256), 0, st, p, sh);
            else hipLaunchKernelGGL((in_bwd_finalize2_kernel<bf16_t, 2>), grid, dim3(256), 0, st, p, sh);
        }
        return rs_check_launch();
    }
    if (dtype == RS_F32) hipLaunchKernelGGL(in_bwd_finalize_kernel<float>, dim3(blocks, p.N), dim3(256), 0, st, p);
    else hipLaunchKernelGGL(in_bwd_finalize_kernel<bf16_t>, dim3(blocks, p.N), dim3(256), 0, st, p);
    return rs_check_launch();
}

int rs_launch_pool(const PoolParams& p, int dtype, int bwd, int blocks, hipStream_t st) {
    const int KP = dtype == RS_F32 ? 4 : 8;
    const int CV = p.C / KP;
    if (CV > 256) return RS_ERR_UNSUPPORTED;
    if (!bwd) {
        const size_t smem = (size_t)(256 / CV) * p.C * 2 * sizeof(float);
        if (rs_glue_variant(-1) && (size_t)blocks * p.N < 1024) {
            const int z = stat_csplit(blocks, p.N, CV);
            const dim3 grid(blocks, p.N, z), blk(z == 1 ? 256 : (CV / z) * (256 / CV));
            if (dtype == RS_F32) hipLaunchKernelGGL((maxpool_fwd2_kernel<float, 4>), grid, blk, smem / z, st, p);
            else hipLaunchKernelGGL((maxpool_fwd2_kernel<bf16_t, 4>), grid, blk, smem / z, st, p);
        } else {
            if (dtype == RS_F32) hipLaunchKernelGGL(maxpool_fwd_kernel<float>, dim3(blocks, p.N), dim3(256), smem, st, p);
            else hipLaunchKernelGGL(maxpool_fwd_kernel<bf16_t>, dim3(blocks, p.N), dim3(256), smem, st, p);
        }
    } else {
        const size_t items = (size_t)(p.D / 2) * (p.H / 2) * (p.W / 2) * CV;
        int b = rs_elem_blocks(items), threads = 256;
        if (rs_glue_variant(-1) && (size_t)b * p.N < 512) { threads = 64; b = (int)((items + 63) / 64); }
        if (dtype == RS_F32) hipLaunchKernelGGL(maxpool_bwd_kernel<float>, dim3(b, p.N), dim3(threads), 0, st, p);
        else hipLaunchKernelGGL(maxpool_bwd_kernel<bf16_t>, dim3(b, p.N), dim3(threads), 0, st, p);
    }
    return rs_check_launch();
}

int rs_launch_subsample(const PoolParams& p, int dtype, int bwd, int blocks, hipStream_t st) {
    const int KP = dtype == RS_F32 ? 4 : 8;
    const int CV = p.C / KP;
    if (CV > 256) return RS_ERR_UNSUPPORTED;
    if (!bwd) {
        const size_t smem = (size_t)(256 / CV) * p.C * 2 * sizeof(float);
        const int z = stat_csplit(blocks, p.N, CV);
        const dim3 grid(blocks, p.N, z), blk(z == 1 ? 256 : (CV / z) * (256 / CV));
        if (dtype == RS_F32) hipLaunchKernelGGL(subsample_fwd_kernel<float>, grid, blk, smem / z, st, p);
        else hipLaunchKernelGGL(subsample_fwd_kernel<bf16_t>, grid, blk, smem / z, st, p);
    } else {
        const int b = rs_elem_blocks((size_t)p.D * p.H * p.W * CV);
        if (dtype == RS_F32) hipLaunchKernelGGL(subsample_bwd_kernel<float>, dim3(b, p.N), dim3(256), 0, st, p);
        else hipLaunchKernelGGL(subsample_bwd_kernel<bf16_t>, dim3(b, p.N), dim3(256), 0, st, p);
    }
    return rs_check_launch();
}

static int launch_upsample_bwd4(const void* g, int ldg, void* dx, int lddx, int N, int ID, int IH, int IW, int OD, int OH, int OW, int C, hipStream_t st) {
    static const bool off = getenv("RSUPER_UPSAMPLE_BWD4") && atoi(getenv("RSUPER_UPSAMPLE_BWD4")) == 0;
    if (off || (C % 8) || N > 65535) return RS_ERR_UNSUPPORTED;
    if ((size_t)OD * OH * OW * (size_t)ldg * 2 >= 0xFFFFFFFFull) return RS_ERR_UNSUPPORTED;
    struct Memo { int k[6]; int ok, nmax; };
    static thread_local Memo memo[8] = {};
    static thread_local int memo_next = 0;
    const int key[6] = {ID, IH, IW, OD, OH, OW};
    const Memo* hit = nullptr;
    for (int i = 0; i < 8 && !hit; ++i) if (memo[i].k[0] && !memcmp(memo[i].k, key, sizeof(key))) hit = &memo[i];
    if (!hit) {
        Memo& m = memo[memo_next++ & 7];
        memcpy(m.k, key, sizeof(key));
        m.ok = up_pair_window(ID, OD) <= UP4_ROWS && up_pair_window(IH, OH) <= UP4_ROWS;
        m.nmax = up_max_count(IW, OW);
        hit = &m;
    }
    if (!hit->ok) return RS_ERR_UNSUPPORTED;
    const int nmax = hit->nmax;
    if (nmax > 6) return RS_ERR_UNSUPPORTED;
    UpInParams p = {g, ldg, dx, lddx, N, ID, IH, IW, OD, OH, OW, C};
    const int nbx = (IW * (C / 8) + 255) / 256;
    const unsigned blocks = (unsigned)(((ID + 1) / 2) * ((IH + 1) / 2) * nbx);
    if (nmax <= 4) hipLaunchKernelGGL((upsample_bwd4_kernel<4>), dim3(blocks, N), dim3(256), 0, st, p, nbx);
    else hipLaunchKernelGGL((upsample_bwd4_kernel<6>), dim3(blocks, N), dim3(256), 0, st, p, nbx);
    return rs_check_launch();
}

int rs_launch_upsample(const UpParams& p, int dtype, int bwd, int blocks, hipStream_t st) {
    const int KP = dtype == RS_F32 ? 4 : 8;
    const int CV = p.C / KP;
    if (CV > 256) return RS_ERR_UNSUPPORTED;
    if (!bwd) {
        static const bool v1 = getenv("RSUPER_UPSAMPLE_V1") != nullptr;
        const size_t smem = (size_t)(256 / CV) * p.C * 2 * sizeof(float);
        const bool small = (size_t)p.N * p.ID * p.IH * p.IW * p.ldx < 0x7FFFFFFFull;
        const size_t tab3 = (size_t)(p.OD + p.OH + p.OW) * sizeof(UpTab);
        const bool fwd3 = rs_glue_variant(-1) && small && (size_t)p.ID * p.IH * p.IW * p.ldx * (dtype == RS_F32 ? 4 : 2) < 0xFFFFFFFFull && smem + tab3 <= 64 * 1024;
        if (v1 || !small) {
            if (dtype == RS_F32) hipLaunchKernelGGL(upsample_fwd_kernel<float>, dim3(blocks, p.N), dim3(256), smem, st, p);
            else hipLaunchKernelGGL(upsample_fwd_kernel<bf16_t>, dim3(blocks, p.N), dim3(256), smem, st, p);
        } else if (fwd3) {
            const int z = stat_csplit(blocks, p.N, CV);
            const dim3 grid(blocks, p.N, z), blk(z == 1 ? 256 : (CV / z) * (256 / CV));
            if (dtype == RS_F32) hipLaunchKernelGGL(upsample_fwd3_kernel<float>, grid, blk, smem / z + tab3, st, p);
            else hipLaunchKernelGGL(upsample_fwd3_kernel<bf16_t>, grid, blk, smem / z + tab3, st, p);
        } else {
            if (dtype == RS_F32) hipLaunchKernelGGL(upsample_fwd2_kernel<float>, dim3(blocks, p.N), dim3(256), smem, st, p);
            else hipLaunchKernelGGL(upsample_fwd2_kernel<bf16_t>, dim3(blocks, p.N), dim3(256), smem, st, p);
        }
    } else {
        static const bool v1 = getenv("RSUPER_UPSAMPLE_V1") != nullptr;
        auto ratio = [](int O, int I) { return I > 1 ? (double)(O - 1) / (double)(I - 1) : (double)O; };
        const double rmax = fmax(ratio(p.OD, p.ID), fmax(ratio(p.OH, p.IH), ratio(p.OW, p.IW)));
        if (!v1 && 2.0 * rmax + 2.0 > (double)UP_MAXW + 1e-9) return RS_ERR_UNSUPPORTED;
        const int b = rs_elem_blocks((size_t)p.ID * p.IH * p.IW * CV);
        const size_t tab = (size_t)(p.ID + p.IH + p.IW) * sizeof(UpEnt);
        const bool small = (size_t)p.OD * p.OH * p.OW * p.ldy * (dtype == RS_F32 ? 4 : 2) < 0xFFFFFFFFull && (size_t)p.ID * p.IH * p.IW * CV < 0xFFFFFFFFull && tab <= 48 * 1024;
        if (!v1 && dtype == RS_BF16) {
            const int rc = launch_upsample_bwd4(p.y, p.ldy, p.dx, p.lddx, p.N, p.ID, p.IH, p.IW, p.OD, p.OH, p.OW, p.C, st);
            if (rc != RS_ERR_UNSUPPORTED) return rc;
        }
        if (v1 || !small) {
            if (dtype == RS_F32) hipLaunchKernelGGL(upsample_bwd_kernel<float>, dim3(b, p.N), dim3(256), 0, st, p);
            else hipLaunchKernelGGL(upsample_bwd_kernel<bf16_t>, dim3(b, p.N), dim3(256), 0, st, p);
        } else {
            if (dtype == RS_F32) hipLaunchKernelGGL(upsample_bwd2_kernel<float>, dim3(b, p.N), dim3(256), tab, st, p);
            else hipLaunchKernelGGL(upsample_bwd2_kernel<bf16_t>, dim3(b, p.N), dim3(256), tab, st, p);
        }
    }
    return rs_check_launch();
}

#define RS_DISPATCH_C(KERNEL, T, C, ...)                                                        \
    switch (C) {                                                                                \
        case 8: { auto k = KERNEL<T, 8>; set_smem(k, smem); hipLaunchKernelGGL(k, __VA_ARGS__); break; }   \
        case 16: { auto k = KERNEL<T, 16>; set_smem(k, smem); hipLaunchKernelGGL(k, __VA_ARGS__); break; } \
        case 32: { auto k = KERNEL<T, 32>; set_smem(k, smem); hipLaunchKernelGGL(k, __VA_ARGS__); break; } \
        case 64: { auto k = KERNEL<T, 64>; set_smem(k, smem); hipLaunchKernelGGL(k, __VA_ARGS__); break; } \
        default: return RS_ERR_UNSUPPORTED;                                                     \
    }

static float* small_ws(int which) {
    static float* ws[16][2] = {};
    int dev = 0;
    if (hipGetDevice(&dev) != hipSuccess || dev < 0 || dev >= 16) return nullptr;
    if (!ws[dev][which] && hipMalloc((void**)&ws[dev][which], (size_t)SMALL_WS_BLOCKS * SMALL_WS_ROW * sizeof(float)) != hipSuccess) return nullptr;
    return ws[dev][which];
}

int rs_launch_stem(const StemParams& p, int dtype, int wgrad, hipStream_t st) {
    const int vox = p.D * p.H * p.W;
    if (!wgrad) {
        const size_t smem = (size_t)(256 * (p.C + 1)) * sizeof(float);
        dim3 grid((vox + 255) / 256, p.N);
        if (p.C <= 32 && (p.C % 4) == 0) {
            if (dtype == RS_F32) hipLaunchKernelGGL(stem_fwd_mfma_kernel<float>, grid, dim3(256), 0, st, p);
            else hipLaunchKernelGGL(stem_fwd_mfma_kernel<bf16_t>, grid, dim3(256), 0, st, p);
            return rs_check_launch();
        }
        if (dtype == RS_F32) { RS_DISPATCH_C(stem_fwd_kernel, float, p.C, grid, dim3(256), smem, st, p) }
        else { RS_DISPATCH_C(stem_fwd_kernel, bf16_t, p.C, grid, dim3(256), smem, st, p) }
    } else {
        HeadParams hp{};
        const long items = (long)p.N * ((vox + 255) / 256);
        dim3 grid((unsigned)(items < SMALL_WS_BLOCKS ? items : SMALL_WS_BLOCKS));
        float* ws = small_ws(0);
        if (!ws) return RS_ERR_LAUNCH;
        const size_t smem = (size_t)(256 * 33 + 256 * 29) * sizeof(float);
// ... 46 lines not shown
```

r-super_amd/hip/lib.py:

```python
import ctypes
import os
from ctypes import c_int, c_long, c_longlong, c_size_t, c_float, c_double, c_void_p, c_uint32, c_uint, c_ulonglong

_HERE = os.path.dirname(os.path.abspath(__file__))
SO_PATH = os.path.join(os.path.dirname(_HERE), 'csrc', 'librsuper_hip.so')

F32, BF16 = 0, 1
BLUR_MAX_RADIUS = 5
GENESIS_MAX_BOXES, GENESIS_MAX_BLOCK_SIDE, GENESIS_MAX_AXIS = 5, 16, 169
_LIB = None

P = c_void_p
_SIGS = {
    'rsuper_version': (ctypes.c_char_p, []),
    'rsuper_device_check': (c_int, []),
    'rsuper_conv3_packed_elems': (c_size_t, [c_int] * 5),
    'rsuper_conv3_pack_weights': (c_int, [c_int, c_int, P, P, c_int, c_int, c_int, c_int, c_int, P, P]),
    'rsuper_conv3_pack_weights_batch': (c_int, [c_int, c_int, P, P, P, P, P, P]),
    'rsuper_conv3_tiles': (c_int, [c_int] * 3),
    'rsuper_conv3_variant': (c_int, [c_int]),
    'rsuper_conv3_wgrad2_min_tiles': (c_int, [c_int]),
    'rsuper_conv3_plan': (c_int, [c_int] * 11 + [P]),
    'rsuper_conv3_box_bn': (c_int, [c_int] * 6),
    'rsuper_conv3_kd_bn': (c_int, [c_int] * 8),
    'rsuper_conv3_set_workspace': (c_int, [P, c_size_t]),
    'rsuper_conv3_workspace_bytes': (c_size_t, []),
    'rsuper_conv3_wgrad_plan': (c_int, [c_int] * 12 + [P]),
    'rsuper_conv3_wgrad_splits': (c_int, [c_int] * 9),
    'rsuper_conv3_part_rows': (c_int, [c_int] * 9),
    'rsuper_conv3_s2_part_rows': (c_int, [c_int] * 9),
    'rsuper_conv3_igemm_s2': (c_int, [c_int, c_int, P, c_int, c_int, P, P, c_int, c_int, P, c_int, c_int, c_int, c_int, c_int, P, c_int, P, P, c_int, P, P]),
    'rsuper_conv3_igemm': (c_int, [c_int, c_int, P, c_int, c_int, P, P, c_int, c_int, P, P, c_int, c_int, c_int, c_int, c_int, c_int,
                                   P, c_int, P, c_int, P, P, c_int, c_int, P, P, c_int, c_int, P, P]),
    'rsuper_conv3_igemm_split_out': (c_int, [c_int, c_int, P, c_int, c_int, P, P, c_int, c_int, P, P, c_int, c_int, c_int, c_int, c_int, c_int,
                                             P, c_int, P, c_int, P, P, c_int, c_int, P, P, c_int, c_int, P, c_int, c_longlong, P]),
    'rsuper_conv3_wgrad': (c_int, [c_int, c_int, P, c_int, c_int, P, P, c_int, c_int, P, P, c_int, c_int, P, c_int, c_int,
                                   P, P, P, c_int, c_int, c_int, c_int, c_int, P]),
    'rsuper_conv3_wgrad_partial': (c_int, [c_int, c_int, P, c_int, c_int, P, P, c_int, c_int, P, P, c_int, c_int, P, c_int, c_int,
                                           P, c_int, c_int, c_int, c_int, c_int, P]),
    'rsuper_conv3_wgrad_reduce': (c_int, [P, c_int, c_int, c_int, c_int, P, P, P]),
    'rsuper_conv3_wgrad_reduce_batch': (c_int, [c_int, P, P, P, P, P, P, P, P]),
    'rsuper_conv3_wgrad_reduce_batch_stats': (c_int, [c_int, P, P, P, P, P, P, P, c_int, P, P, P, P, P, P, P, P, c_float, P]),
    'rsuper_conv3_wgrad_s2_splits': (c_int, [c_int] * 7),
    'rsuper_conv3_wgrad_s2': (c_int, [c_int, P, c_int, c_int, P, P, c_int, c_int, P, c_int, c_int, P, P, P, c_int, c_int, c_int, c_int, c_int, P]),
    'rsuper_pointwise_packed_bytes': (c_size_t, [c_int, c_int, c_int]),
    'rsuper_pointwise': (c_int, [c_int, c_int, P, c_int, P, P, P, c_int, P, c_int, c_long, c_int, c_int, P, P]),
    'rsuper_pointwise_pack_batch': (c_int, [c_int, P, c_int, c_long, P, P]),
    'rsuper_pointwise_wgrad_splits': (c_int, [c_long, c_int, c_int]),
    'rsuper_pointwise_wgrad': (c_int, [c_int, P, c_int, P, c_int, c_long, c_int, c_int, P, c_int, P, P, P]),
    'rsuper_stats_finalize': (c_int, [P, c_int, c_int, c_int, c_double, c_float, c_int, c_int, P, P]),
    'rsuper_glue_variant': (c_int, [c_int]),
    'rsuper_in_bwd_finalize': (c_int, [c_int, P, c_int, P, c_int, P, P, P, c_int, P, c_int, P, c_int, c_int, c_int, c_int, P]),
    'rsuper_maxpool2_fwd': (c_int, [c_int, P, c_int, P, c_int, P, c_int, c_int, c_int, c_int, c_int, c_int, P]),
    'rsuper_maxpool2_bwd': (c_int, [c_int, P, c_int, P, c_int, P, c_int, c_int, c_int, c_int, c_int, c_int, P]),
    'rsuper_maxpool2_bwd_add': (c_int, [c_int, P, c_int, P, c_int, P, c_int, P, c_int, c_int, c_int, c_int, c_int, c_int, P]),
    'rsuper_subsample2_fwd': (c_int, [c_int, P, c_int, P, c_int, P, c_int, c_int, c_int, c_int, c_int, c_int, P]),
    'rsuper_subsample2_bwd': (c_int, [c_int, P, c_int, P, c_int, c_int, c_int, c_int, c_int, c_int, P]),
    'rsuper_upsample_fwd': (c_int, [c_int, P, c_int, P, c_int, P, c_int] + [c_int] * 8 + [P]),
    'rsuper_upsample_bwd': (c_int, [c_int, P, c_int, P, c_int] + [c_int] * 8 + [P]),
    'rsuper_stem_fwd': (c_int, [c_int, P, P, P, c_int, P, c_int, c_int, c_int, c_int, c_int, P]),
    'rsuper_stem_wgrad': (c_int, [c_int, P, P, c_int, P, c_int, c_int, c_int, c_int, c_int, P]),
    'rsuper_head_fwd': (c_int, [c_int, P, c_int, P, P, P, c_int, c_int, c_int, c_int, P]),
    'rsuper_head_bwd_data': (c_int, [c_int, P, P, P, c_int, c_int, c_int, c_int, c_int, P]),
    'rsuper_head_bwd_weight': (c_int, [c_int, P, c_int, P, P, P, c_int, c_int, c_int, c_int, P]),
    'rsuper_head_bwd': (c_int, [c_int, P, c_int, P, P, P, c_int, P, P, c_int, c_int, c_int, c_int, P]),
    'rsuper_plane_partials_fwd': (c_int, [P, c_size_t, P, P, P, P, P, c_int, c_int, c_size_t, P]),
    'rsuper_plane_partials_fwd2': (c_int, [P, c_size_t, P, P, c_int, c_int, P, P, P, P, P, c_int, c_int, c_size_t, P]),
    'rsuper_plane_partials_fwd3': (c_int, [P, c_size_t, P, P, c_int, c_int, P, P, P, P, P, c_int, c_int, c_size_t, P]),
    'rsuper_plane_partials_blocks': (c_int, [c_size_t]),
    'rsuper_plane_sums_reduce': (c_int, [P, c_int, c_int, P, P]),
    'rsuper_plane_partials_bwd2': (c_int, [P, c_size_t, P, P, c_int, c_int, P, P, P, P, P, P, c_int, c_int, c_size_t, P]),
    'rsuper_cnorm_rows': (c_int, [c_long]),
    'rsuper_cnorm_small': (c_int, [P, P, P, P, P, c_int, c_long, c_int, c_int, c_float, c_int, P]),
    'rsuper_cnorm_forward': (c_int, [P, P, P, P, c_int, c_long, c_int, c_int, c_float, P]),
    'rsuper_cnorm_backward': (c_int, [P, P, P, P, P, P, c_int, c_long, c_int, c_int, P]),
    'rsuper_cnorm_stats': (c_int, [P, P, P, P, c_int, c_long, c_int, c_int, c_int, P]),
    'rsuper_cnorm_apply': (c_int, [P, P, P, P, P, c_int, c_long, c_int, c_int, c_int, P]),
    'rsuper_token_attn_supported': (c_int, [c_int, c_int]),
    'rsuper_token_attn_fwd': (c_int, [P, P, P, c_int, c_int, c_int, c_int, c_float, P]),
    'rsuper_token_attn_bwd': (c_int, [P, P, P, P, P, c_int, c_int, c_int, c_int, c_float, P]),
    'rsuper_battn_supported': (c_int, [c_int, c_int, c_int]),
    'rsuper_battn_chunks': (c_int, [c_int, c_int]),
    'rsuper_battn_fwd': (c_int, [P] * 7 + [c_int] * 5 + [c_float, P]),
    'rsuper_battn_bwd': (c_int, [P] * 9 + [c_int] * 5 + [c_float, P]),
    'rsuper_se_forward': (c_int, [P] * 10 + [c_int, c_long, c_int, c_int, P]),
    'rsuper_se_backward': (c_int, [P] * 17 + [c_int, c_long, c_int, c_int, P]),
    'rsuper_cl_planar': (c_int, [P, P, c_int, c_long, c_int, c_int, c_int, P]),
    'rsuper_depthwise3_rows': (c_int, [c_long]),
    'rsuper_depthwise3_fwd': (c_int, [P, P, P, c_int, c_int, c_int, c_int, c_int, c_int, P]),
    'rsuper_depthwise3_wgrad': (c_int, [P, P, P, P, c_int, c_int, c_int, c_int, c_int, P]),
    'rsuper_seg_from_sums': (c_int, [P, P, c_int, c_int, c_size_t, c_double, P, P, P]),
    'rsuper_report_from_sums': (c_int, [P, P, c_int, c_int, c_int, c_size_t, c_int, P, P, c_double, c_double, c_int, P, c_int, c_int, P, P, P]),
    'rsuper_plane_partials_bwd': (c_int, [P, c_size_t, P, P, P, P, P, P, c_int, c_int, c_size_t, P]),
    'rsuper_sigmoid_mask': (c_int, [P, P, P, c_size_t, P]),
    'rsuper_window_accumulate': (c_int, [P, P] + [c_int] * 11 + [P]),
    'rsuper_window_normalize': (c_int, [P, P, P, P, c_long, c_int, c_int, c_int, P]),
    'rsuper_dilate_volume': (c_int, [P, P, P, c_long, c_int, c_int, c_int, c_int, P]),
    'rsuper_dilate_volume_sparse': (c_int, [P, P, P, P, c_long, c_int, c_int, c_int, c_int, P]),
    'rsuper_ball_workspace_floats': (c_long, [c_int, c_int, c_int, c_int]),
    'rsuper_ball_conv_argmax': (c_int, [P, c_int, c_int, c_int, c_int, c_float, P, P, P, P]),
    'rsuper_insert_ball': (c_int, [P, c_int, c_int, c_int, c_int, c_int, c_int, c_int, c_int, P, P]),
    'rsuper_insert_ball_at': (c_int, [P, c_int, c_int, c_int, P, c_int, c_int, P, P]),
    'rsuper_radix_hist': (c_int, [P, P, c_long, c_uint32, c_int, P, P]),
    'rsuper_topk_mark': (c_int, [P, P, c_long, c_uint32, c_uint, P, P]),
    'rsuper_compact': (c_int, [P, P, c_long, P, P, P, P]),
    'rsuper_rank_weights': (c_int, [P, P, c_uint, c_float, c_float, P, P]),
    'rsuper_rank_assign': (c_int, [P, c_uint, c_float, c_float, P, P]),
    'rsuper_topk_select': (c_int, [P, P, c_long, c_uint, P, P, P]),
    'rsuper_topk_select_multi': (c_int, [P, P, c_long, P, c_int, P, P, c_int, P]),
    'rsuper_plane_any': (c_int, [P, c_long, c_long, P, P]),
    'rsuper_guard_range': (c_int, [P, c_size_t, c_float, c_float, P, P]),
    'rsuper_guard_consistency': (c_int, [P, P, P, c_int, c_int, P, P]),
    'rsuper_mask_op': (c_int, [P, P, c_long, c_int, P]),
    'rsuper_unpack_bits': (c_int, [P, P, c_int, c_int, c_int, c_long, P]),
    'rsuper_pack_bits': (c_int, [P, P, c_int, c_int, c_long, c_long, c_long, P]),
    'rsuper_timer_event_create': (c_int, [P]),
    'rsuper_timer_event_record': (c_int, [P, P]),
    'rsuper_timer_event_elapsed_ms': (c_int, [P, P, P]),
    'rsuper_timer_event_destroy': (c_int, [P]),
    'rsuper_unpack_bits_sel': (c_int, [P, P, c_int, c_int, c_int, c_long, P, P, P]),
    'rsuper_plane_any_bits': (c_int, [P, c_int, c_int, c_int, c_long, P, P]),
    'rsuper_zero_where': (c_int, [P, P, c_long, P]),
    'rsuper_count': (c_int, [P, c_long, P, P]),
    'rsuper_detection_workspace_bytes': (c_long, [c_int]),
    'rsuper_detection': (c_int, [P, c_int, c_int, c_int, c_int, c_int, c_int, c_int, P, c_int, c_int, P, P, P, P]),
    'rsuper_detection_binary': (c_int, [P, c_int, c_int, c_int, c_int, c_int, c_int, c_int, c_int, c_double, c_int, P, P, P]),
    'rsuper_organ_mask_u8': (c_int, [P, c_int, c_int, c_int, c_int, c_int, P, P, P, P, P]),
    'rsuper_organ_mask_f32': (c_int, [P, c_int, c_int, c_int, c_int, c_int, P, P, P, P, P]),
    'rsuper_largest_component_workspace_bytes': (c_long, [c_int, c_int, c_int]),
    'rsuper_largest_component': (c_int, [P, c_int, c_int, c_int, c_int, P, P, P]),
    'rsuper_lesion_candidates_workspace_bytes': (c_long, [c_int] * 4),
    'rsuper_lesion_candidates_begin': (c_int, [P, c_int, c_int, c_int, c_int, P, P, P]),
    'rsuper_lesion_candidates_run': (c_int, [P, P, c_int, c_int, c_int, c_int, c_float, c_int, c_float, P, P, c_int, P]),
    'rsuper_affine_crop': (c_int, [P, P, P, c_int, c_int, c_int, c_int, c_int, c_int, P, P, P, c_int, c_int, c_int, P, P]),
    'rsuper_intensity_augment_workspace_bytes': (c_long, [c_int] * 4),
    'rsuper_intensity_augment_launches': (c_int, [c_int, P]),
    'rsuper_intensity_augment': (c_int, [P, P, c_int, c_int, c_int, c_int, P, P, P, P, P, P, P, c_long, P]),
    'rsuper_genesis_workspace_bytes': (c_long, [c_int] * 5),
# ... 77 lines not shown
```

r-super_amd/hip/library.py:

```python
import torch

from . import ops as _ops

LIB = torch.library.Library('rsuper', 'DEF')


class _Ctx:
    needs_input_grad = ()

    def save_for_backward(self, *ts):
        pass

    def mark_non_differentiable(self, *ts):
        pass

    def set_materialize_grads(self, v):
        pass


def _register_plain(name, schema, fn):
    LIB.define(name + schema)
    LIB.impl(name, fn, 'CUDA')
    return getattr(torch.ops.rsuper, name)


def _register(name, schema, Fn, to_fn_args=None):
    LIB.define(name + schema)

    def kernel(*args):
        c = _Ctx()
        c.needs_input_grad = (False,) * 16
        return Fn.forward(c, *(to_fn_args(*args) if to_fn_args else args))

    def with_autograd(*args):
        return Fn.apply(*(to_fn_args(*args) if to_fn_args else args))

    LIB.impl(name, kernel, 'CUDA')
    LIB.impl(name, with_autograd, 'AutogradCUDA')
    return getattr(torch.ops.rsuper, name)


class _Apply:

    def __init__(self, op, adapt=None, doc=None):
        self.op, self.adapt, self.__doc__ = op, adapt, doc

    def apply(self, *args):
        return self.op(*(self.adapt(*args) if self.adapt else args))


def _bb_fn_args(xa, mra, xb, mrb, w1, w2, ws, pack_bufs, pack_bns, stride):
    return xa, mra, xb, mrb, w1, w2, ws, (None if pack_bufs is None else (list(pack_bufs), list(pack_bns))), stride


def _bb_apply_args(xa, mra, xb, mrb, w1, w2, ws, packs=None, stride=1):
    return xa, mra, xb, mrb, w1, w2, ws, (None if packs is None else list(packs[0])), (None if packs is None else list(packs[1])), stride


def install():
    if getattr(_ops, '_LIBRARY_INSTALLED', False):
        return
    reg = [
        ('BasicBlockFn', 'basic_block',
         '(Tensor xa, Tensor mra, Tensor? xb, Tensor? mrb, Tensor w1, Tensor w2, Tensor? ws, Tensor[]? pack_bufs, int[]? pack_bns, int stride) -> (Tensor, Tensor)',
         _bb_fn_args, _bb_apply_args),
        ('MaxPoolFn', 'maxpool2', '(Tensor x) -> (Tensor, Tensor)', None, None),
        ('MaxPoolSkipFn', 'maxpool2_skip', '(Tensor(a) x) -> (Tensor, Tensor, Tensor(a))', None, None),
        ('UpsampleFn', 'upsample_trilinear', '(Tensor x, int[] size) -> (Tensor, Tensor)', lambda x, size: (x, tuple(size)), None),
        ('StemFn', 'stem_conv', '(Tensor img, Tensor w, ScalarType dtype) -> (Tensor, Tensor)', None, None),
        ('HeadFn', 'head_conv', '(Tensor x, Tensor w, Tensor b) -> Tensor', None, None),
        ('Conv3Fn', 'conv3', '(Tensor x, Tensor w) -> Tensor', None, None),
        ('PlanarFn', 'cl_planar', '(Tensor x, int K) -> Tensor', None, None),
        ('SqueezeExciteFn', 'squeeze_excite', '(Tensor x, Tensor w1, Tensor b1, Tensor w2, Tensor b2) -> Tensor', None, None),
        ('BidirAttnFn', 'bidir_attention', '(Tensor fqv, Tensor mqv, int heads, float scale) -> (Tensor, Tensor)', None, None),
        ('TokenAttnFn', 'token_attention', '(Tensor qkv, int heads, float scale) -> Tensor', None, None),
        ('ChannelNormFn', 'channel_norm', '(Tensor x, float eps, bool relu) -> Tensor', None, None),
        ('DepthwiseConvFn', 'depthwise_conv3', '(Tensor x, Tensor w) -> Tensor', None, None),
        ('ClsTailFn', 'cls_tail', '(Tensor x, Tensor reducer_w, Tensor reducer_b, Tensor norm1_w, Tensor norm1_b, Tensor qkv_w, Tensor out_w, Tensor out_b, '
         'Tensor norm2_w, Tensor norm2_b, Tensor fc1_w, Tensor fc1_b, Tensor fc2_w, Tensor fc2_b, Tensor head_w, Tensor head_b) -> Tensor', None, None),
        ('InfoNceFn', 'info_nce', '(Tensor query, Tensor positive_key, float temperature) -> Tensor', None, None),
        ('ClsLossFn', 'classification_loss', '(Tensor logits, Tensor flags_label, Tensor? flags_mask, Tensor? flags_unk, Tensor? weights, int class_set) '
         '-> Tensor', None, None),
    ]
    for cls, name, schema, to_fn, adapt in reg:
        Fn = getattr(_ops, cls)
        op = _register(name, schema, Fn, to_fn)
        setattr(_ops, '_' + cls, Fn)
        setattr(_ops, cls, _Apply(op, adapt, Fn.__doc__))
    _ops._LIBRARY_INSTALLED = True


def install_loss_ops(lf):
    if getattr(lf, '_LIBRARY_INSTALLED', False):
        return

    def pp_to_fn(logits, x_off, xstride, planes, kinv, t, k, w1, w2, kflags, tpk, tpk_classes):
        from ..training.dataset.packed import PackedBits
        return logits, [lf._Term(x_off[i], xstride[i], planes[i], t[i], k[i], w1[i], w2[i], kinv[i], kflags[i],
                                 None if tpk[i] is None else PackedBits(tpk[i], tpk_classes[i])) for i in range(len(planes))]

    def pp_adapt(logits, terms):
        return (logits, [tm.x_off for tm in terms], [tm.xstride for tm in terms], [tm.planes for tm in terms], [tm.kinv for tm in terms],
                [tm.t for tm in terms], [tm.k for tm in terms], [tm.w1 for tm in terms], [tm.w2 for tm in terms], [tm.kflags for tm in terms],
                [None if tm.tpk is None else tm.tpk.packed for tm in terms], [0 if tm.tpk is None else tm.tpk.C for tm in terms])

    pp = _register('plane_partials', '(Tensor logits, int[] x_off, int[] xstride, int[] planes, bool[] kinv, Tensor?[] t, Tensor?[] k, '
                   'Tensor?[] w1, Tensor?[] w2, Tensor?[] kflags, Tensor?[] tpk, int[] tpk_classes) -> (Tensor, Tensor)', lf._PartialsFn, pp_to_fn)
    sf = _register('seg_from_sums', '(Tensor sums, Tensor? cw, int B, int C, int V, float scale) -> Tensor', lf._SegFromSums)
    dv = _register_plain('dilate_volume', '(Tensor vol, int kernel_size) -> Tensor', _ops.dilate_volume)
    bs = _register_plain('ball_search', '(Tensor x, int diameter, float sigma) -> Tensor', _ops.ball_search)
    lf._PartialsFnImpl, lf._SegFromSumsImpl = lf._PartialsFn, lf._SegFromSums
    lf._PartialsFn = _Apply(pp, pp_adapt, lf._PartialsFnImpl.__doc__)
    lf._SegFromSums = _Apply(sf, None, lf._SegFromSumsImpl.__doc__)
    _ops._dilate_volume_impl, _ops._ball_search_impl = _ops.dilate_volume, _ops.ball_search
    _ops.dilate_volume, _ops.ball_search = dv, bs
    lf._LIBRARY_INSTALLED = True


_PLAIN_GROUPS = {}


def _install_plain(group, ops):
    if group not in _PLAIN_GROUPS:
        _PLAIN_GROUPS[group] = tuple(_register_plain(name, schema, fn) for name, schema, fn in ops)
    return _PLAIN_GROUPS[group]


def install_postprocess_ops(detection_volumes, detection_binary, organ_mask, largest_component):
    return _install_plain('postprocess', (
        ('detection_volumes', '(Tensor x, int[] out_shape, float[] thresholds, bool erode, Tensor? workspace=None) -> (Tensor, Tensor)', detection_volumes),
        ('detection_binary', '(Tensor x, int[] out_shape, float th, bool erode, Tensor? workspace=None) -> Tensor', detection_binary),
        ('organ_mask', '(Tensor pred, int[] lesion, int[] organ_a, int[] organ_b) -> Tensor', organ_mask),
        ('largest_component', '(Tensor mask, Tensor? workspace=None) -> Tensor', largest_component)))


def install_augment_ops(affine_crop):
    return _install_plain('augment', (
        ('affine_crop', '(Tensor img, Tensor[] volumes, Tensor theta, int[] out_size, int[] offsets) -> (Tensor, Tensor[])', affine_crop),))[0]


def install_crop_ops(class_counts, select_voxel, crop_box):
    return _install_plain('crop', (
        ('class_counts', '(Tensor packed, int C, bool plain, Tensor? workspace=None) -> (Tensor, Tensor)', class_counts),
        ('select_voxel', '(Tensor packed, int C, bool plain, Tensor table, int b, int column, int k, int count, int[] add) -> Tensor', select_voxel),
        ('crop_box', '(Tensor? img, Tensor[] volumes, int[] size, int[] pad, Tensor? center, int[] origin) -> (Tensor, Tensor[], Tensor)', crop_box)))


def install_report_crop_ops(union_bbox, union_bits, bits_open, label_remap):
    return _install_plain('report_crop', (
        ('union_bbox', '(Tensor packed, int C, bool plain, int[] sets) -> Tensor', union_bbox),
        ('union_bits', '(Tensor packed, int C, bool plain, int b, int set, int[] box) -> Tensor', union_bits),
# ... 50 lines not shown
```

r-super_amd/hip/ops.py:

```python
import ctypes
import os

import torch
import torch.nn.functional as F

from . import lib as _l

EPS = 1e-4
_DT = {torch.float32: _l.F32, torch.bfloat16: _l.BF16}


def use_tr():
    return int(os.environ.get('RSUPER_WGRAD_TR', '1'))


_DEV_INDEX = None


def _stream():
    global _DEV_INDEX
    if _DEV_INDEX is None:
        _DEV_INDEX = torch.cuda.current_device()
    return torch._C._cuda_getCurrentRawStream(_DEV_INDEX)

# ... 501 lines not shown
        dy1 = in_bwd_finalize(Src(g1), y1, gm1, Cout)
        sa = Src(xa, mr=mra)
        tiles = _L().rsuper_conv3_tiles(D, H, W)
        g0 = torch.empty((N, D, H, W, Ca), device=dev, dtype=dt)
        if strided_kernel():
            wpd1 = pack_weights(dt, 1, w1, ws, Cout, Cout, Ca, 0, 64)
            part0 = torch.empty((N, _L().rsuper_conv3_s2_part_rows(_DT[dt], 2, Cout, Cout, Ca, N, D, H, W), Ca, 2), device=dev, dtype=torch.float32)
            igemm_s2(2, Src(dy1), sdo, wpd1, Ca, dims, g0, part0, ea=sa)
            gm0 = stats_finalize(part0, D * H * W, mode=1)
            dw1, dws = grad_dest(w1), grad_dest(ws)
            wgrad_s2(sa, Src(dy1), sdo, dw1, dws, dims)
        else:
            dfull = torch.empty((N, D, H, W, 2 * Cout), device=dev, dtype=dt)
            subsample2_scatter(dy1, dfull, 0, dims)
            subsample2_scatter(dout, dfull, Cout, dims)
            bnd = pick_bn(Ca, dt, tiles * N, dims, epi=1)
            wpd1 = pack_weights(dt, 1, w1, ws, Cout, Cout, Ca, 0, bnd)
            part0 = part_buffer(dt, dims, Ca, bnd, dev, epi=1)
            igemm(1, Src(dfull, C=Cout), Src(dfull, C=Cout, off=Cout), wpd1, Ca, bnd, dims, g0, part=part0, ea=sa)
            gm0 = stats_finalize(part0, D * H * W, mode=1)
            dw1, dws = grad_dest(w1), grad_dest(ws)
            wgrad(sa, None, Src(dfull, C=Cout), Src(dfull, C=Cout, off=Cout), dw1, dws, dims)
        dxa = in_bwd_finalize(Src(g0), sa, gm0, Ca)
        return dxa, None, None, None, dw1, dw2, dws, None, None

    @staticmethod
    def backward(ctx, dout, _unused):
        if ctx.stride == 2:
            return _BB._backward_s2(ctx, dout)
        try:
            return _BB._backward_s1(ctx, dout)
        except BaseException:
            del _DEFERRED[:]
            raise

    @staticmethod
    def _backward_s1(ctx, dout):
        xa, mra, xb, mrb, ys, mr_y1, w1, w2, ws = ctx.saved_tensors
        dout = dout.contiguous()
        N, D, H, W, Ca = xa.shape
        Cb = 0 if xb is None else xb.shape[-1]
        Cin, Cout = Ca + Cb, w1.shape[0]
        has_sc = ws is not None
        dims = (N, D, H, W)
        dev, dt = xa.device, xa.dtype
        tiles = _L().rsuper_conv3_tiles(D, H, W)
        cnt = D * H * W
        y1 = Src(ys, C=Cout, mr=mr_y1)
        sdo = Src(dout)
        if ctx.packs is not None:
            bpk = (ctx.packs[0][2:], ctx.packs[1][2:])
        else:
            bufs, bbns = block_packs(w1, w2, ws, Ca, Cb, dt, tiles * N, True, dims)
            bpk = (bufs[2:], bbns[2:])
        bn, wpd2 = bpk[1][0], bpk[0][0]
        g1 = torch.empty((N, D, H, W, Cout), device=dev, dtype=dt)
        part = part_buffer(dt, dims, Cout, bn, dev, epi=1)
        igemm(1, sdo, None, wpd2, Cout, bn, dims, g1, part=part, ea=y1)
        gm1 = stats_finalize(part, cnt, mode=1)
        dw2 = grad_dest(w2)
        wgrad(y1, None, sdo, None, dw2, None, dims, defer=True)
        dy1 = in_bwd_finalize(Src(g1), y1, gm1, Cout)
        sa = Src(xa, mr=mra)
        sb = None if xb is None else Src(xb, mr=mrb)
        sdo1 = sdo if has_sc else None
        if len(bpk[0]) == 3:
            g0s = [Src(torch.empty((N, D, H, W, Ca), device=dev, dtype=dt)), Src(torch.empty((N, D, H, W, Cb), device=dev, dtype=dt))]
            stats = []
            for g, src, wp_, bn in ((g0s[0], sa, bpk[0][1], bpk[1][1]), (g0s[1], sb, bpk[0][2], bpk[1][2])):
                part0 = part_buffer(dt, dims, src.C, bn, dev, epi=1)
                igemm(1, Src(dy1), sdo1, wp_, src.C, bn, dims, g.t, part=part0, ea=src)
                stats.append((part0, cnt, 1, 0))
        else:
            g0 = torch.empty((N, D, H, W, Cin), device=dev, dtype=dt)
            g0s = [Src(g0, C=Ca), Src(g0, C=Cb, off=Ca)]
            bn, wpd1 = bpk[1][1], bpk[0][1]
            part0 = part_buffer(dt, dims, Cin, bn, dev, epi=1)
            igemm(1, Src(dy1), sdo1, wpd1, Cin, bn, dims, g0, part=part0, ea=sa, eb=sb)
            stats = [(part0, cnt, 1, Ca if xb is not None else 0)]
        dw1 = grad_dest(w1)
        dws = grad_dest(ws) if has_sc else None
        wgrad(sa, sb, Src(dy1), sdo1, dw1, dws, dims, defer=True)
        gm0 = flush_wgrad_reduces(stats=stats)
        if xb is None:
            dxa, dxb = in_bwd_finalize(g0s[0], sa, gm0[0], Ca, add1=None if has_sc else dout), None
        else:
            gma, gmb = gm0 if len(gm0) == 2 else gm0[0]
            dxa, dxb = in_bwd_finalize(g0s[0], sa, gma, Ca), in_bwd_finalize(g0s[1], sb, gmb, Cb)
        return dxa, None, dxb, None, dw1, dw2, dws, None, None


_BB = BasicBlockFn


def _stat_blocks(ovox):
    return max(1, min(2048, ovox // 64))


class MaxPoolFn(torch.autograd.Function):

    @staticmethod
    def forward(ctx, x):
        _chk_act(x)
        N, D, H, W, C = x.shape
        OD, OH, OW = D // 2, H // 2, W // 2
        y = torch.empty((N, OD, OH, OW, C), device=x.device, dtype=x.dtype)
        blocks = _stat_blocks(OD * OH * OW)
        part = torch.empty((N, blocks, C, 2), device=x.device, dtype=torch.float32)
        _l.check(_L().rsuper_maxpool2_fwd(_DT[x.dtype], _ptr(x), C, _ptr(y), C, _ptr(part), blocks, N, D, H, W, C, _stream()), 'maxpool2_fwd')
        mr = stats_finalize(part, OD * OH * OW)
        ctx.save_for_backward(x)
        ctx.mark_non_differentiable(mr)
        ctx.set_materialize_grads(False)
        return y, mr

    @staticmethod
    def backward(ctx, dy, _unused):
        (x,) = ctx.saved_tensors
        dy = dy.contiguous()
        N, D, H, W, C = x.shape
        dx = torch.empty_like(x)
        _l.check(_L().rsuper_maxpool2_bwd(_DT[x.dtype], _ptr(x), C, _ptr(dy), C, _ptr(dx), C, N, D, H, W, C, _stream()), 'maxpool2_bwd')
        return dx


_MaxPoolFn = MaxPoolFn


class MaxPoolSkipFn(torch.autograd.Function):

    @staticmethod
    def forward(ctx, x):
        y, mr = _MaxPoolFn.forward(ctx, x)
        return y, mr, x.view_as(x)

    @staticmethod
    def backward(ctx, dy, _unused, dskip):
        if dy is None:
            return dskip
        if dskip is None:
            return _MaxPoolFn.backward(ctx, dy, None)
        (x,) = ctx.saved_tensors
        N, D, H, W, C = x.shape
        dy, dskip = dy.contiguous(), dskip.contiguous()
        dx = torch.empty_like(x)
        rc = _L().rsuper_maxpool2_bwd_add(_DT[x.dtype], _ptr(x), C, _ptr(dy), C, _ptr(dskip), C, _ptr(dx), C, N, D, H, W, C, _stream())
        if rc == 3:
            return _MaxPoolFn.backward(ctx, dy, None) + dskip
        _l.check(rc, 'maxpool2_bwd_add')
        return dx


def subsample2(x, with_stats=True):
    N, D, H, W, C = x.shape
    OD, OH, OW = (D + 1) // 2, (H + 1) // 2, (W + 1) // 2
    y = torch.empty((N, OD, OH, OW, C), device=x.device, dtype=x.dtype)
    blocks = _stat_blocks(OD * OH * OW)
    part = torch.empty((N, blocks, C, 2), device=x.device, dtype=torch.float32) if with_stats else None
    _l.check(_L().rsuper_subsample2_fwd(_DT[x.dtype], _ptr(x), C, _ptr(y), C, _ptr(part), blocks, N, D, H, W, C, _stream()), 'subsample2_fwd')
    return y, (stats_finalize(part, OD * OH * OW) if with_stats else None)


def subsample2_scatter(dy, out, off, dims):
    N, D, H, W = dims
    C = dy.shape[-1]
    _l.check(_L().rsuper_subsample2_bwd(_DT[dy.dtype], _ptr(dy), C, _ptr(out, off), out.shape[-1], N, D, H, W, C, _stream()), 'subsample2_bwd')


class UpsampleFn(torch.autograd.Function):

    @staticmethod
    def forward(ctx, x, size):
        _chk_act(x)
        N, ID, IH, IW, C = x.shape
        OD, OH, OW = size
        y = torch.empty((N, OD, OH, OW, C), device=x.device, dtype=x.dtype)
        blocks = _stat_blocks(OD * OH * OW)
        part = torch.empty((N, blocks, C, 2), device=x.device, dtype=torch.float32)
        _l.check(_L().rsuper_upsample_fwd(_DT[x.dtype], _ptr(x), C, _ptr(y), C, _ptr(part), blocks, N, ID, IH, IW, OD, OH, OW, C, _stream()),
                  'upsample_fwd')
        mr = stats_finalize(part, OD * OH * OW)
        ctx.in_shape = tuple(x.shape)
        ctx.mark_non_differentiable(mr)
        ctx.set_materialize_grads(False)
        return y, mr

    @staticmethod
    def backward(ctx, dy, _unused):
        dy = dy.contiguous()
        N, ID, IH, IW, C = ctx.in_shape
        OD, OH, OW = dy.shape[1:4]
        dx = torch.empty(ctx.in_shape, device=dy.device, dtype=dy.dtype)
        _l.check(_L().rsuper_upsample_bwd(_DT[dy.dtype], _ptr(dy), C, _ptr(dx), C, N, ID, IH, IW, OD, OH, OW, C, _stream()), 'upsample_bwd')
        return dx, None


class StemFn(torch.autograd.Function):

    @staticmethod
    def forward(ctx, img, w, dtype):
        assert img.dim() == 5 and img.shape[1] == 1, 'hot path supports in_chan == 1 (reference configs use 1)'
        img = img.contiguous().float()
        N, _, D, H, W = img.shape
        C = w.shape[0]
        y = torch.empty((N, D, H, W, C), device=img.device, dtype=dtype)
        blocks = -(-(D * H * W) // 256)
        part = torch.empty((N, blocks, C, 2), device=img.device, dtype=torch.float32)
        _l.check(_L().rsuper_stem_fwd(_DT[dtype], _ptr(img), _ptr(w), _ptr(y), C, _ptr(part), N, D, H, W, C, _stream()), 'stem_fwd')
        mr = stats_finalize(part, D * H * W)
        ctx.save_for_backward(img, w)
        ctx.mark_non_differentiable(mr)
        ctx.set_materialize_grads(False)
        return y, mr

    @staticmethod
    def backward(ctx, dy, _unused):
        img, w = ctx.saved_tensors
        dy = dy.contiguous()
        N, _, D, H, W = img.shape
        C = w.shape[0]
        dw = grad_dest(w)
        _l.check(_L().rsuper_stem_wgrad(_DT[dy.dtype], _ptr(img), _ptr(dy), C, _ptr(dw), N, D, H, W, C, _stream()), 'stem_wgrad')
        return None, dw, None


class HeadFn(torch.autograd.Function):

    @staticmethod
    def forward(ctx, x, w, b):
        _chk_act(x)
        N, D, H, W, C = x.shape
        K = w.shape[0]
        logits = torch.empty((N, K, D, H, W), device=x.device, dtype=torch.float32)
        _l.check(_L().rsuper_head_fwd(_DT[x.dtype], _ptr(x), C, _ptr(w), _ptr(b), _ptr(logits), N, D * H * W, C, K, _stream()), 'head_fwd')
        ctx.save_for_backward(x, w, b)
        return logits

    @staticmethod
    def backward(ctx, dl):
        x, w, b = ctx.saved_tensors
        dl = dl.contiguous().float()
        N, D, H, W, C = x.shape
        K = w.shape[0]
        dx = torch.empty_like(x)
        dw = grad_dest(w)
        db = grad_dest(b)
        st = _stream()
        _l.check(_L().rsuper_head_bwd(_DT[x.dtype], _ptr(x), C, _ptr(dl), _ptr(w), _ptr(dx), C, _ptr(dw), _ptr(db), N, D * H * W, C, K, st), 'head_bwd')
        return dx, dw, db


class Conv3Fn(torch.autograd.Function):

    @staticmethod
    def forward(ctx, x, w):
        _chk_act(x)
        N, D, H, W, Cin = x.shape
        Cout = w.shape[0]
        assert tuple(w.shape[1:]) == (Cin, 3, 3, 3) and Cout % 8 == 0 and w.dtype == torch.float32
        dt, dims = x.dtype, (N, D, H, W)
        tiles = _L().rsuper_conv3_tiles(D, H, W) * N
        bn = pick_bn(Cout, dt, tiles, dims, epi=0)
        wc = w.contiguous()
        out = torch.empty((N, D, H, W, Cout), device=x.device, dtype=dt)
        igemm(0, Src(x), None, pack_weights(dt, 0, wc, None, Cin, 0, Cout, 0, bn), Cout, bn, dims, out)
        ctx.save_for_backward(x, wc)
        return out

    @staticmethod
    def backward(ctx, dout):
        x, w = ctx.saved_tensors
        N, D, H, W, Cin = x.shape
        Cout = w.shape[0]
        dt, dims = x.dtype, (N, D, H, W)
        dout = dout.contiguous()
        dx = dw = None
        if ctx.needs_input_grad[0]:
# ... 494 lines not shown
```

r-super_amd/model/dim3/unet.py:

```python
import os

import torch
import torch.nn as nn

from .conv_layers import BasicBlock
from .unet_utils import inconv, down_block, up_block
from ...hip import ops, lib as _lib


def _get_block(name):
    if name != 'BasicBlock':
        raise NotImplementedError(f"block={name!r}: the gfx950 hot path implements 'BasicBlock' (config/abdomenatlas/resunet_3d.yaml:13)")
    return BasicBlock


class UNet(nn.Module):
    def __init__(self, in_ch, base_ch, scale=[2, 2, 2, 2], kernel_size=[3, 3, 3, 3, 3], num_classes=1, block='BasicBlock',
                 pool=True, norm='in', compute_dtype=None):
        super().__init__()
        if norm != 'in':
            raise NotImplementedError("norm must be 'in' (InstanceNorm3d) on the gfx950 hot path")
        if in_ch != 1 or base_ch % 8:
            raise NotImplementedError('in_ch must be 1 and base_ch a multiple of 8')
        if base_ch not in (8, 16, 32, 64) or num_classes > 256:
            raise NotImplementedError('the stem / head kernels are instantiated for base_ch 8 / 16 / 32 / 64 and hold the weights of up to 256 classes '
                                      'in LDS (reference configs: base 32, 26-42 classes)')
        blk = _get_block(block)
        num_block = 2
        ks = [k if isinstance(k, (list, tuple)) else [k] * 3 for k in kernel_size]
        b = base_ch
        self.inc = inconv(in_ch, b, block=blk, kernel_size=ks[0], norm=norm)
        self.down1 = down_block(b, 2 * b, num_block, blk, ks[1], scale[0], pool, norm)
        self.down2 = down_block(2 * b, 4 * b, num_block, blk, ks[2], scale[1], pool, norm)
        self.down3 = down_block(4 * b, 8 * b, num_block, blk, ks[3], scale[2], pool, norm)
        self.down4 = down_block(8 * b, 10 * b, num_block, blk, ks[4], scale[3], pool, norm)
        self.up1 = up_block(10 * b, 8 * b, num_block, blk, ks[3], scale[3], norm)
        self.up2 = up_block(8 * b, 4 * b, num_block, blk, ks[2], scale[2], norm)
        self.up3 = up_block(4 * b, 2 * b, num_block, blk, ks[1], scale[1], norm)
        self.up4 = up_block(2 * b, b, num_block, blk, ks[0], scale[0], norm)
        self.outc = nn.Conv3d(b, num_classes, kernel_size=1)
        self.compute_dtype = compute_dtype or os.environ.get('RSUPER_DTYPE', 'bf16')
        self.pool = bool(pool)

    def _dtype(self):
        return {'bf16': torch.bfloat16, 'f32': torch.float32}[self.compute_dtype]

    def forward(self, x):
        if not x.is_cuda:
            raise _lib.RSuperHipError('rsuper_amd UNet runs on MI355X only (no CPU fallback); move the input to cuda')
        _lib.require_device()
        dt = self._dtype()
        x1, m1 = self.inc(x, dt)
        x2, m2, x1 = self.down1(x1, m1, True)
        x3, m3, x2 = self.down2(x2, m2, True)
        x4, m4, x3 = self.down3(x3, m3, True)
        x5, m5, x4 = self.down4(x4, m4, True)
        o, mo = self.up1(x5, m5, x4, m4)
        o, mo = self.up2(o, mo, x3, m3)
        o, mo = self.up3(o, mo, x2, m2)
        o, mo = self.up4(o, mo, x1, m1)
        logits = ops.HeadFn.apply(o, self.outc.weight, self.outc.bias)
        return {'segmentation': logits}
```

r-super_amd/model/dim3/unet_utils.py:

```python
import torch
import torch.nn as nn

from .conv_layers import BasicBlock
from ...hip import ops


class _Pool(nn.Module):

    def forward(self, x, with_skip=False):
        return ops.MaxPoolSkipFn.apply(x) if with_skip else ops.MaxPoolFn.apply(x)


class inconv(nn.Module):
    def __init__(self, in_ch, out_ch, kernel_size=(3, 3, 3), block=BasicBlock, norm='in'):
        super().__init__()
        self.conv1 = nn.Conv3d(in_ch, out_ch, kernel_size=3, padding=1, bias=False)
        self.conv2 = block(out_ch, out_ch, kernel_size=kernel_size, norm=norm)

    def forward(self, img, dtype):
        x, mr = ops.StemFn.apply(img, self.conv1.weight, dtype)
        return self.conv2(x, mr)


class down_block(nn.Module):
    def __init__(self, in_ch, out_ch, num_block, block=BasicBlock, kernel_size=(3, 3, 3), down_scale=(2, 2, 2), pool=True, norm='in'):
        super().__init__()
        ds = tuple(down_scale) if isinstance(down_scale, (list, tuple)) else (down_scale,) * 3
        if ds != (2, 2, 2):
            raise NotImplementedError('gfx950 hot path implements down_scale (2, 2, 2) (every shipped config)')
        self.pool = bool(pool)
        if pool:
            layers = [_Pool(), block(in_ch, out_ch, kernel_size=kernel_size, norm=norm)]
        else:
            layers = [block(in_ch, out_ch, kernel_size=kernel_size, stride=2, norm=norm)]
        for _ in range(num_block - 1):
            layers.append(block(out_ch, out_ch, kernel_size=kernel_size, norm=norm))
        self.conv = nn.Sequential(*layers)

    def forward(self, x, mr, with_skip=False):
        blocks = list(self.conv)
        skip = x
        if self.pool:
            if with_skip and torch.is_grad_enabled() and x.requires_grad:
                x, mr, skip = blocks[0](x, True)
            else:
                x, mr = blocks[0](x)
            blocks = blocks[1:]
        for blk in blocks:
            x, mr = blk(x, mr)
        return (x, mr, skip) if with_skip else (x, mr)


class up_block(nn.Module):
    def __init__(self, in_ch, out_ch, num_block, block=BasicBlock, kernel_size=(3, 3, 3), up_scale=(2, 2, 2), norm='in'):
        super().__init__()
        layers = [block(in_ch + out_ch, out_ch, kernel_size=kernel_size, norm=norm)]
        for _ in range(num_block - 1):
            layers.append(block(out_ch, out_ch, kernel_size=kernel_size, norm=norm))
        self.conv = nn.Sequential(*layers)

    def forward(self, x1, mr1, x2, mr2):
        up, mru = ops.UpsampleFn.apply(x1, tuple(x2.shape[1:4]))
        x, mr = self.conv[0](x2, mr2, up, mru)
        for blk in list(self.conv)[1:]:
            x, mr = blk(x, mr)
        return x, mr
```

Baseline: 174.2 million voxels/s.

## Fuse instance-norm backward tails into maxpool and upsample backward kernels

Adds lazy variants of the maxpool-with-skip and upsample autograd functions. Their incoming gradients are returned in an un-normalized form along with the per-channel mean/rstd and grad moments, and the instance-norm backward finalize is applied inside the pool/upsample backward kernels rather than in a separate pass. This is meant to cut full-tensor read/write passes over large activation gradients. In exchange it adds extra loads of the saved activation and per-channel constants inside those kernels, and the upsample kernel runs with lower occupancy. By default the maxpool path is enabled (variant 1) and the upsample path only with variant 2.

```diff
diff --git a/include/rsuper_hip.h b/include/rsuper_hip.h
--- a/include/rsuper_hip.h
+++ b/include/rsuper_hip.h
@@ -106,6 +106,11 @@
                         int N, int D, int H, int W, int C, void* stream);
 int rsuper_maxpool2_bwd_add(int dtype, const void* x, int ldx, const void* dy, int lddy, const void* add, int lda, void* dx, int lddx,
                             int N, int D, int H, int W, int C, void* stream);
+int rsuper_maxpool2_bwd_lazy(int dtype, const void* x, int ldx, const void* dy, int lddy, const float* mr_y, const float* gm_y,
+                             const void* add, int lda, const float* mr_x, const float* gm_x, void* dx, int lddx,
+                             int N, int D, int H, int W, int C, void* stream);
+int rsuper_maxpool2_bwd_lazy_plan(int dtype, int N, int D, int H, int W, int C);
+int rsuper_lazy_tails(int v);
 
 int rsuper_subsample2_fwd(int dtype, const void* x, int ldx, void* y, int ldy, float* part, int blocks,
                           int N, int D, int H, int W, int C, void* stream);
@@ -115,6 +120,9 @@
                         int N, int ID, int IH, int IW, int OD, int OH, int OW, int C, void* stream);
 int rsuper_upsample_bwd(int dtype, const void* dy, int lddy, void* dx, int lddx,
                         int N, int ID, int IH, int IW, int OD, int OH, int OW, int C, void* stream);
+int rsuper_upsample_bwd_lazy(int dtype, const void* g, int ldg, const void* u, int ldu, const float* mr, const float* gm, void* dx, int lddx,
+                             int N, int ID, int IH, int IW, int OD, int OH, int OW, int C, void* stream);
+int rsuper_upsample_bwd_lazy_plan(int dtype, int N, int ID, int IH, int IW, int OD, int OH, int OW, int C);
 
 int rsuper_stem_fwd(int dtype, const float* x, const float* w, void* y, int ldy, float* part,
                     int N, int D, int H, int W, int C, void* stream);
diff --git a/r-super_amd/csrc/api.hip b/r-super_amd/csrc/api.hip
--- a/r-super_amd/csrc/api.hip
+++ b/r-super_amd/csrc/api.hip
@@ -20,6 +20,7 @@
 
 #include "igemm_plan.hpp"
 #include "wgrad_plan.hpp"
+#include "lazy_tail_plan.hpp"
 
 template <typename F>
 static int for_chunks(int n, void* const* p, void* const* g, void* const* m, void* const* v, void* const* e, const size_t* numel, F f) {
@@ -421,6 +422,18 @@
     PoolParams p = {x, ldx, (void*)dy, lddy, dx, lddx, nullptr, N, D, H, W, C, add, lda};
     return rs_launch_pool(p, dtype, 1, 1, ST(stream));
 }
+int rsuper_lazy_tails(int v) { return lazy_tails_variant(v); }
+int rsuper_maxpool2_bwd_lazy_plan(int dtype, int N, int D, int H, int W, int C) { return lazy_pool_plan(dtype, N, D, H, W, C); }
+int rsuper_maxpool2_bwd_lazy(int dtype, const void* x, int ldx, const void* dy, int lddy, const float* mr_y, const float* gm_y,
+                             const void* add, int lda, const float* mr_x, const float* gm_x, void* dx, int lddx,
+                             int N, int D, int H, int W, int C, void* stream) {
+    if (!dt_ok(dtype) || !x || !dy || !add || !dx || !ch_ok(C, ldx) || !ch_ok(C, lddy) || !ch_ok(C, lda) || !ch_ok(C, lddx) || C <= 0 || N <= 0 ||
+        D <= 0 || H <= 0 || W <= 0 || (gm_y && !mr_y) || (gm_x && !mr_x))
+        return RS_ERR_ARG;
+    if (lazy_pool_plan(dtype, N, D, H, W, C) != 1) return RS_ERR_UNSUPPORTED;
+    PoolParams p = {x, ldx, (void*)dy, lddy, dx, lddx, nullptr, N, D, H, W, C, add, lda, gm_y ? mr_y : nullptr, gm_y, gm_x ? mr_x : nullptr, gm_x};
+    return rs_launch_pool(p, dtype, 1, 1, ST(stream));
+}
 
 int rsuper_subsample2_fwd(int dtype, const void* x, int ldx, void* y, int ldy, float* part, int blocks,
                           int N, int D, int H, int W, int C, void* stream) {
@@ -445,6 +458,17 @@
     if (!dt_ok(dtype) || !dy || !dx || !ch_ok(C, lddy) || !ch_ok(C, lddx)) return RS_ERR_ARG;
     UpParams p = {nullptr, 0, (void*)dy, lddy, dx, lddx, nullptr, N, ID, IH, IW, OD, OH, OW, C};
     return rs_launch_upsample(p, dtype, 1, 1, ST(stream));
+}
+int rsuper_upsample_bwd_lazy_plan(int dtype, int N, int ID, int IH, int IW, int OD, int OH, int OW, int C) {
+    return lazy_up_plan(dtype, N, ID, IH, IW, OD, OH, OW, C);
+}
+int rsuper_upsample_bwd_lazy(int dtype, const void* g, int ldg, const void* u, int ldu, const float* mr, const float* gm, void* dx, int lddx,
+                             int N, int ID, int IH, int IW, int OD, int OH, int OW, int C, void* stream) {
+    if (!dt_ok(dtype) || !g || !u || !mr || !gm || !dx || !ch_ok(C, ldg) || !ch_ok(C, ldu) || !ch_ok(C, lddx) || C <= 0) return RS_ERR_ARG;
+    const int pl = lazy_up_plan(dtype, N, ID, IH, IW, OD, OH, OW, C);
+    if (pl < 0) return RS_ERR_ARG;
+    if (pl != 1) return RS_ERR_UNSUPPORTED;
+    return rs_launch_upsample_bwd_lazy(g, ldg, u, ldu, mr, gm, dx, lddx, N, ID, IH, IW, OD, OH, OW, C, ST(stream));
 }
 int rsuper_stem_fwd(int dtype, const float* x, const float* w, void* y, int ldy, float* part,
                     int N, int D, int H, int W, int C, void* stream) {
diff --git a/r-super_amd/csrc/lazy_tail_plan.hpp b/r-super_amd/csrc/lazy_tail_plan.hpp
--- /dev/null
+++ b/r-super_amd/csrc/lazy_tail_plan.hpp
@@ -0,0 +1,24 @@
+#pragma once
+#include <stdlib.h>
+#include "common.hpp"
+
+static int lazy_tails_variant(int v) {
+    static int g = getenv("RSUPER_LAZY_TAILS") ? atoi(getenv("RSUPER_LAZY_TAILS")) : 1;
+    if (v >= 0 && v <= 2) g = v;
+    if (g < 0 || g > 2) g = 1;
+    return g;
+}
+
+static int lazy_pool_plan(int dtype, int N, int D, int H, int W, int C) {
+    if (!dt_ok(dtype) || N <= 0 || D <= 0 || H <= 0 || W <= 0 || C <= 0) return -1;
+    if (!lazy_tails_variant(-1)) return 0;
+    const int KP = dtype == RS_F32 ? 4 : 8;
+    if ((D & 1) || (H & 1) || (W & 1) || (C % 8) || C / KP > 256 || N > 65535) return 0;
+    return 1;
+}
+
+static int lazy_up_plan(int dtype, int N, int ID, int IH, int IW, int OD, int OH, int OW, int C) {
+    if (!dt_ok(dtype) || N <= 0 || ID <= 0 || IH <= 0 || IW <= 0 || OD <= 0 || OH <= 0 || OW <= 0 || C <= 0) return -1;
+    if (dtype != RS_BF16 || (C % 8) || N > 65535) return 0;
+    return lazy_tails_variant(-1) == 2;
+}
diff --git a/r-super_amd/csrc/misc.hpp b/r-super_amd/csrc/misc.hpp
--- a/r-super_amd/csrc/misc.hpp
+++ b/r-super_amd/csrc/misc.hpp
@@ -21,6 +21,8 @@
     float* part;
     int N, D, H, W, C;
     const void* add; int lda;
+    const float* mr_y; const float* gm_y;
+    const float* mr_x; const float* gm_x;
 };
 
 struct UpParams {
@@ -74,5 +76,7 @@
 int rs_launch_pool(const PoolParams& p, int dtype, int bwd, int blocks, hipStream_t st);
 int rs_launch_subsample(const PoolParams& p, int dtype, int bwd, int blocks, hipStream_t st);
 int rs_launch_upsample(const UpParams& p, int dtype, int bwd, int blocks, hipStream_t st);
+int rs_launch_upsample_bwd_lazy(const void* g, int ldg, const void* u, int ldu, const float* mr, const float* gm, void* dx, int lddx,
+                                int N, int ID, int IH, int IW, int OD, int OH, int OW, int C, hipStream_t st);
 int rs_launch_stem(const StemParams& p, int dtype, int wgrad, hipStream_t st);
 int rs_launch_head(const HeadParams& p, int dtype, int which, hipStream_t st);
diff --git a/r-super_amd/csrc/unet_misc.hip b/r-super_amd/csrc/unet_misc.hip
--- a/r-super_amd/csrc/unet_misc.hip
+++ b/r-super_amd/csrc/unet_misc.hip
@@ -64,6 +64,20 @@
     }
 }
 
+__device__ __forceinline__ float in_bwd_tail(float g, float x, float mu, float rs, float m1, float m2) {
+    const float xn = (x - mu) * rs;
+    return rs * (g - m1 - xn * m2);
+}
+template <typename T> __device__ __forceinline__ void round_as_stored(float* f) {
+    if constexpr (sizeof(T) == 4) {
+#pragma unroll
+        for (int j = 0; j < Elem<T>::KP; ++j) asm volatile("" : "+v"(f[j]));
+    } else {
+        const uint4 q = pack16<T>(f);
+        unpack16<T>(q, f);
+    }
+}
+
 template <typename T>
 __global__ __launch_bounds__(256) void in_bwd_finalize_kernel(InBwdParams p) {
     constexpr int KP = Elem<T>::KP;
@@ -100,10 +114,7 @@
         unpack16<T>(gq, g);
         unpack16<T>(xq, x);
 #pragma unroll
-        for (int j = 0; j < KP; ++j) {
-            const float xn = (x[j] - mu[j]) * rs[j];
-            o[j] = rs[j] * (g[j] - m1[j] - xn * m2[j]);
-        }
+        for (int j = 0; j < KP; ++j) o[j] = in_bwd_tail(g[j], x[j], mu[j], rs[j], m1[j], m2[j]);
         if (a1p) {
             float a[KP];
             unpack16<T>(a1q, a);
@@ -160,10 +171,7 @@
         unpack16<T>(gq[u], g);
         unpack16<T>(xq[u], x);
 #pragma unroll
-        for (int j = 0; j < KP; ++j) {
-            const float xn = (x[j] - mu[j]) * rs[j];
-            o[j] = rs[j] * (g[j] - m1[j] - xn * m2[j]);
-        }
+        for (int j = 0; j < KP; ++j) o[j] = in_bwd_tail(g[j], x[j], mu[j], rs[j], m1[j], m2[j]);
         if (a1p) {
             float a[KP];
             unpack16<T>(a1q[u], a);
@@ -267,16 +275,32 @@
                                p.part + (((size_t)n * gridDim.x + blockIdx.x) * p.C + (size_t)blockIdx.z * Cb) * 2);
 }
 
-template <typename T>
-__global__ void maxpool_bwd_kernel(PoolParams p) {
+template <typename T, int LAZY>
+__global__ __launch_bounds__(LAZY ? 256 : 1024) void maxpool_bwd_kernel(PoolParams p) {
     constexpr int KP = Elem<T>::KP;
     const int CV = p.C / KP;
     const int n = blockIdx.y;
     const int OD = p.D / 2, OH = p.H / 2, OW = p.W / 2;
     const size_t total = (size_t)OD * OH * OW * CV;
+    constexpr int KY = (LAZY & 1) ? KP : 1, KX = (LAZY & 2) ? KP : 1;
+    [[maybe_unused]] float cy[4][KY], cx[4][KX];
+    [[maybe_unused]] auto constants = [&](int s) {
+#pragma unroll
+        for (int j = 0; j < KP; ++j) {
+            const size_t o = ((size_t)n * p.C + s * KP + j) * 2;
+            if constexpr (LAZY & 1) { cy[0][j] = p.mr_y[o]; cy[1][j] = p.mr_y[o + 1]; cy[2][j] = p.gm_y[o]; cy[3][j] = p.gm_y[o + 1]; }
+            if constexpr (LAZY & 2) { cx[0][j] = p.mr_x[o]; cx[1][j] = p.mr_x[o + 1]; cx[2][j] = p.gm_x[o]; cx[3][j] = p.gm_x[o + 1]; }
+        }
+    };
+    const bool fixed_slot = LAZY != 0 && (blockDim.x % CV) == 0;
+    if constexpr (LAZY != 0) {
+        const size_t i0 = (size_t)blockIdx.x * blockDim.x + threadIdx.x;
+        if (fixed_slot && i0 < total) constants((int)(i0 % CV));
+    }
     for (size_t i = (size_t)blockIdx.x * blockDim.x + threadIdx.x; i < total; i += (size_t)gridDim.x * blockDim.x) {
         const int s = (int)(i % CV); const int v = (int)(i / CV);
         const int ow = v % OW, oh = (v / OW) % OH, od = v / (OW * OH);
+        if constexpr (LAZY != 0) { if (!fixed_slot) constants(s); }
         float x[8][KP], m[KP], dy[KP];
 #pragma unroll
         for (int j = 0; j < KP; ++j) m[j] = -INFINITY;
@@ -288,6 +312,11 @@
             for (int j = 0; j < KP; ++j) m[j] = fmaxf(m[j], x[k][j]);
         }
         unpack16<T>(*(const uint4*)((const T*)p.y + ((size_t)n * OD * OH * OW + v) * p.ldy + s * KP), dy);
+        if constexpr (LAZY & 1) {
+#pragma unroll
+            for (int j = 0; j < KP; ++j) dy[j] = in_bwd_tail(dy[j], m[j], cy[0][j], cy[1][j], cy[2][j], cy[3][j]);
+            round_as_stored<T>(dy);
+        }
         bool done[KP];
 #pragma unroll
         for (int j = 0; j < KP; ++j) done[j] = false;
@@ -304,6 +333,11 @@
             if (p.add) {
                 float a[KP];
                 unpack16<T>(*(const uint4*)((const T*)p.add + ((((size_t)n * p.D + d) * p.H + h) * p.W + w) * (size_t)p.lda + s * KP), a);
+                if constexpr (LAZY & 2) {
+#pragma unroll
+                    for (int j = 0; j < KP; ++j) a[j] = in_bwd_tail(a[j], x[k][j], cx[0][j], cx[1][j], cx[2][j], cx[3][j]);
+                    round_as_stored<T>(a);
+                }
 #pragma unroll
                 for (int j = 0; j < KP; ++j) o[j] += a[j];
             }
@@ -767,13 +801,15 @@
     const void* g; int ldg;
     void* dx; int lddx;
     int N, ID, IH, IW, OD, OH, OW, C;
+    const void* u; int ldu;
+    const float* mr; const float* gm;
 };
 #ifndef UP4_SL
 #define UP4_SL 2
 #endif
 constexpr int UP4_ROWS = 16;
-template <int NT>
-__global__ __launch_bounds__(256, 3) void upsample_bwd4_kernel(UpInParams p, int nbx) {
+template <int NT, bool LAZY>
+__global__ __launch_bounds__(256, LAZY ? 2 : 3) void upsample_bwd4_kernel(UpInParams p, int nbx) {
     typedef bf16_t T;
     constexpr int CPT = 8, NWD = CPT / 2;
     constexpr int SL = UP4_SL;
@@ -846,6 +882,21 @@
 #pragma unroll
         for (int k = 0; k < CPT; ++k) acc[i][k] = 0.f;
     uint4 gq[SL][NT];
+    const uint32_t urow = LAZY ? (uint32_t)p.ldu * 2u : 0u;
+    const __amdgpu_buffer_rsrc_t urs = __builtin_amdgcn_make_buffer_rsrc(LAZY ? (void*)((const T*)p.u + (size_t)n * ovox * p.ldu) : nullptr, 0,
+                                                                         LAZY ? ovox * urow : 0u, 0x00020000);
+    [[maybe_unused]] uint32_t uoff[LAZY ? NT : 1];
+    [[maybe_unused]] uint4 uq[LAZY ? SL : 1][LAZY ? NT : 1];
+    [[maybe_unused]] float cmu[LAZY ? CPT : 1], crs[LAZY ? CPT : 1], cm1[LAZY ? CPT : 1], cm2[LAZY ? CPT : 1];
+    if constexpr (LAZY) {
+#pragma unroll
+        for (int c = 0; c < NT; ++c) uoff[c] = (uint32_t)(wlo + (wc[c] != 0.f ? c : 0)) * urow + (uint32_t)s * 16u;
+#pragma unroll
+        for (int k = 0; k < CPT; ++k) {
+            const size_t o = ((size_t)n * p.C + s * CPT + k) * 2;
+            cmu[k] = p.mr[o]; crs[k] = p.mr[o + 1]; cm1[k] = p.gm[o]; cm2[k] = p.gm[o + 1];
+        }
+    }
     int ia = 0, ib = 0;
     auto issue = [&](int slot) {
         const uint32_t row = (uint32_t)__builtin_amdgcn_readfirstlane(((od0 + ia) * p.OH + (oh0 + ib)) * p.OW);
@@ -853,6 +904,10 @@
         for (int c = 0; c < NT; ++c) {
             const auto q = __builtin_amdgcn_raw_buffer_load_b128(grs, goff[c], row * grow, 0);
             gq[slot][c] = make_uint4(q[0], q[1], q[2], q[3]);
+            if constexpr (LAZY) {
+                const auto r = __builtin_amdgcn_raw_buffer_load_b128(urs, uoff[c], row * urow, 0);
+                uq[slot][c] = make_uint4(r[0], r[1], r[2], r[3]);
+            }
         }
         if (++ib == rh) { ib = 0; ++ia; }
     };
@@ -870,7 +925,16 @@
 #pragma unroll
             for (int c = 0; c < NT; ++c) {
                 const f32x2_t w2 = {wc[c], wc[c]};
-                const uint32_t wq[4] = {gq[h][c].x, gq[h][c].y, gq[h][c].z, gq[h][c].w};
+                uint4 gv = gq[h][c];
+                if constexpr (LAZY) {
+                    float g[CPT], x[CPT];
+                    unpack16<T>(gv, g);
+                    unpack16<T>(uq[h][c], x);
+#pragma unroll
+                    for (int k = 0; k < CPT; ++k) g[k] = in_bwd_tail(g[k], x[k], cmu[k], crs[k], cm1[k], cm2[k]);
+                    gv = pack16<T>(g);
+                }
+                const uint32_t wq[4] = {gv.x, gv.y, gv.z, gv.w};
 #pragma unroll
                 for (int j = 0; j < NWD; ++j) {
                     const f32x2_t v2 = {__uint_as_float(wq[j] << 16), __uint_as_float(wq[j] & 0xffff0000u)};
@@ -1381,8 +1445,15 @@
         const size_t items = (size_t)(p.D / 2) * (p.H / 2) * (p.W / 2) * CV;
         int b = rs_elem_blocks(items), threads = 256;
         if (rs_glue_variant(-1) && (size_t)b * p.N < 512) { threads = 64; b = (int)((items + 63) / 64); }
-        if (dtype == RS_F32) hipLaunchKernelGGL(maxpool_bwd_kernel<float>, dim3(b, p.N), dim3(threads), 0, st, p);
-        else hipLaunchKernelGGL(maxpool_bwd_kernel<bf16_t>, dim3(b, p.N), dim3(threads), 0, st, p);
+        const int lazy = (p.gm_y ? 1 : 0) | (p.gm_x ? 2 : 0);
+        if ((p.gm_y && !p.mr_y) || (p.gm_x && (!p.mr_x || !p.add))) return RS_ERR_ARG;
+#define RS_POOL_BWD(LZ)                                                                                                   \
+        case LZ:                                                                                                          \
+            if (dtype == RS_F32) hipLaunchKernelGGL((maxpool_bwd_kernel<float, LZ>), dim3(b, p.N), dim3(threads), 0, st, p);   \
+            else hipLaunchKernelGGL((maxpool_bwd_kernel<bf16_t, LZ>), dim3(b, p.N), dim3(threads), 0, st, p);             \
+            break;
+        switch (lazy) { RS_POOL_BWD(0) RS_POOL_BWD(1) RS_POOL_BWD(2) RS_POOL_BWD(3) }
+#undef RS_POOL_BWD
     }
     return rs_check_launch();
 }
@@ -1405,10 +1476,12 @@
     return rs_check_launch();
 }
 
-static int launch_upsample_bwd4(const void* g, int ldg, void* dx, int lddx, int N, int ID, int IH, int IW, int OD, int OH, int OW, int C, hipStream_t st) {
+static int launch_upsample_bwd4(const void* g, int ldg, void* dx, int lddx, int N, int ID, int IH, int IW, int OD, int OH, int OW, int C, hipStream_t st,
+                                const UpInParams* lz = nullptr) {
     static const bool off = getenv("RSUPER_UPSAMPLE_BWD4") && atoi(getenv("RSUPER_UPSAMPLE_BWD4")) == 0;
     if (off || (C % 8) || N > 65535) return RS_ERR_UNSUPPORTED;
     if ((size_t)OD * OH * OW * (size_t)ldg * 2 >= 0xFFFFFFFFull) return RS_ERR_UNSUPPORTED;
+    if (lz && (size_t)OD * OH * OW * (size_t)lz->ldu * 2 >= 0xFFFFFFFFull) return RS_ERR_UNSUPPORTED;
     struct Memo { int k[6]; int ok, nmax; };
     static thread_local Memo memo[8] = {};
     static thread_local int memo_next = 0;
@@ -1426,11 +1499,26 @@
     const int nmax = hit->nmax;
     if (nmax > 6) return RS_ERR_UNSUPPORTED;
     UpInParams p = {g, ldg, dx, lddx, N, ID, IH, IW, OD, OH, OW, C};
+    if (lz) { p.u = lz->u; p.ldu = lz->ldu; p.mr = lz->mr; p.gm = lz->gm; }
     const int nbx = (IW * (C / 8) + 255) / 256;
     const unsigned blocks = (unsigned)(((ID + 1) / 2) * ((IH + 1) / 2) * nbx);
-    if (nmax <= 4) hipLaunchKernelGGL((upsample_bwd4_kernel<4>), dim3(blocks, N), dim3(256), 0, st, p, nbx);
-    else hipLaunchKernelGGL((upsample_bwd4_kernel<6>), dim3(blocks, N), dim3(256), 0, st, p, nbx);
+    if (lz) {
+        if (nmax <= 4) hipLaunchKernelGGL((upsample_bwd4_kernel<4, true>), dim3(blocks, N), dim3(256), 0, st, p, nbx);
+        else hipLaunchKernelGGL((upsample_bwd4_kernel<6, true>), dim3(blocks, N), dim3(256), 0, st, p, nbx);
+    } else {
+        if (nmax <= 4) hipLaunchKernelGGL((upsample_bwd4_kernel<4, false>), dim3(blocks, N), dim3(256), 0, st, p, nbx);
+        else hipLaunchKernelGGL((upsample_bwd4_kernel<6, false>), dim3(blocks, N), dim3(256), 0, st, p, nbx);
+    }
     return rs_check_launch();
+}
+
+int rs_launch_upsample_bwd_lazy(const void* g, int ldg, const void* u, int ldu, const float* mr, const float* gm, void* dx, int lddx,
+                                int N, int ID, int IH, int IW, int OD, int OH, int OW, int C, hipStream_t st) {
+    static const bool v1 = getenv("RSUPER_UPSAMPLE_V1") != nullptr;
+    if (v1) return RS_ERR_UNSUPPORTED;
+    UpInParams lz = {};
+    lz.u = u; lz.ldu = ldu; lz.mr = mr; lz.gm = gm;
+    return launch_upsample_bwd4(g, ldg, dx, lddx, N, ID, IH, IW, OD, OH, OW, C, st, &lz);
 }
 
 int rs_launch_upsample(const UpParams& p, int dtype, int bwd, int blocks, hipStream_t st) {
diff --git a/r-super_amd/hip/lib.py b/r-super_amd/hip/lib.py
--- a/r-super_amd/hip/lib.py
+++ b/r-super_amd/hip/lib.py
@@ -54,6 +54,11 @@
     'rsuper_maxpool2_fwd': (c_int, [c_int, P, c_int, P, c_int, P, c_int, c_int, c_int, c_int, c_int, c_int, P]),
     'rsuper_maxpool2_bwd': (c_int, [c_int, P, c_int, P, c_int, P, c_int, c_int, c_int, c_int, c_int, c_int, P]),
     'rsuper_maxpool2_bwd_add': (c_int, [c_int, P, c_int, P, c_int, P, c_int, P, c_int, c_int, c_int, c_int, c_int, c_int, P]),
+    'rsuper_maxpool2_bwd_lazy': (c_int, [c_int, P, c_int, P, c_int, P, P, P, c_int, P, P, P, c_int, c_int, c_int, c_int, c_int, c_int, P]),
+    'rsuper_maxpool2_bwd_lazy_plan': (c_int, [c_int] * 6),
+    'rsuper_lazy_tails': (c_int, [c_int]),
+    'rsuper_upsample_bwd_lazy': (c_int, [c_int, P, c_int, P, c_int, P, P, P, c_int] + [c_int] * 8 + [P]),
+    'rsuper_upsample_bwd_lazy_plan': (c_int, [c_int] * 9),
     'rsuper_subsample2_fwd': (c_int, [c_int, P, c_int, P, c_int, P, c_int, c_int, c_int, c_int, c_int, c_int, P]),
     'rsuper_subsample2_bwd': (c_int, [c_int, P, c_int, P, c_int, c_int, c_int, c_int, c_int, c_int, P]),
     'rsuper_upsample_fwd': (c_int, [c_int, P, c_int, P, c_int, P, c_int] + [c_int] * 8 + [P]),
diff --git a/r-super_amd/hip/library.py b/r-super_amd/hip/library.py
--- a/r-super_amd/hip/library.py
+++ b/r-super_amd/hip/library.py
@@ -66,7 +66,9 @@
          _bb_fn_args, _bb_apply_args),
         ('MaxPoolFn', 'maxpool2', '(Tensor x) -> (Tensor, Tensor)', None, None),
         ('MaxPoolSkipFn', 'maxpool2_skip', '(Tensor(a) x) -> (Tensor, Tensor, Tensor(a))', None, None),
+        ('MaxPoolSkipLazyFn', 'maxpool2_skip_lazy', '(Tensor(a) x, Tensor(b) mrx) -> (Tensor, Tensor, Tensor(a), Tensor(b))', None, None),
         ('UpsampleFn', 'upsample_trilinear', '(Tensor x, int[] size) -> (Tensor, Tensor)', lambda x, size: (x, tuple(size)), None),
+        ('UpsampleLazyFn', 'upsample_trilinear_lazy', '(Tensor x, int[] size) -> (Tensor, Tensor)', lambda x, size: (x, tuple(size)), None),
         ('StemFn', 'stem_conv', '(Tensor img, Tensor w, ScalarType dtype) -> (Tensor, Tensor)', None, None),
         ('HeadFn', 'head_conv', '(Tensor x, Tensor w, Tensor b) -> Tensor', None, None),
         ('Conv3Fn', 'conv3', '(Tensor x, Tensor w) -> Tensor', None, None),
diff --git a/r-super_amd/hip/ops.py b/r-super_amd/hip/ops.py
--- a/r-super_amd/hip/ops.py
+++ b/r-super_amd/hip/ops.py
@@ -607,12 +607,23 @@
         dws = grad_dest(ws) if has_sc else None
         wgrad(sa, sb, Src(dy1), sdo1, dw1, dws, dims, defer=True)
         gm0 = flush_wgrad_reduces(stats=stats)
+        lazy_a, lazy_b = ctx.needs_input_grad[1] and has_sc, xb is not None and ctx.needs_input_grad[3]
         if xb is None:
-            dxa, dxb = in_bwd_finalize(g0s[0], sa, gm0[0], Ca, add1=None if has_sc else dout), None
+            gma, gmb = gm0[0], None
         else:
             gma, gmb = gm0 if len(gm0) == 2 else gm0[0]
-            dxa, dxb = in_bwd_finalize(g0s[0], sa, gma, Ca), in_bwd_finalize(g0s[1], sb, gmb, Cb)
-        return dxa, None, dxb, None, dw1, dw2, dws, None, None
+
+        def raw(g):
+            return g.t if g.C == g.ld else g.t[..., g.off:g.off + g.C]
+        if lazy_a:
+            dxa = raw(g0s[0])
+        else:
+            dxa, gma = in_bwd_finalize(g0s[0], sa, gma, Ca, add1=None if has_sc else dout), None
+        if lazy_b:
+            dxb = raw(g0s[1])
+        else:
+            dxb, gmb = (None if xb is None else in_bwd_finalize(g0s[1], sb, gmb, Cb)), None
+        return dxa, gma, dxb, gmb, dw1, dw2, dws, None, None
 
 
 _BB = BasicBlockFn
@@ -622,18 +633,41 @@
     return max(1, min(2048, ovox // 64))
 
 
+def _maxpool_fwd(x):
+    _chk_act(x)
+    N, D, H, W, C = x.shape
+    OD, OH, OW = D // 2, H // 2, W // 2
+    y = torch.empty((N, OD, OH, OW, C), device=x.device, dtype=x.dtype)
+    blocks = _stat_blocks(OD * OH * OW)
+    part = torch.empty((N, blocks, C, 2), device=x.device, dtype=torch.float32)
+    _l.check(_L().rsuper_maxpool2_fwd(_DT[x.dtype], _ptr(x), C, _ptr(y), C, _ptr(part), blocks, N, D, H, W, C, _stream()), 'maxpool2_fwd')
+    return y, stats_finalize(part, OD * OH * OW)
+
+
+def _maxpool_bwd(x, dy):
+    dy = dy.contiguous()
+    N, D, H, W, C = x.shape
+    dx = torch.empty_like(x)
+    _l.check(_L().rsuper_maxpool2_bwd(_DT[x.dtype], _ptr(x), C, _ptr(dy), C, _ptr(dx), C, N, D, H, W, C, _stream()), 'maxpool2_bwd')
+    return dx
+
+
+def _maxpool_bwd_add(x, dy, dskip):
+    N, D, H, W, C = x.shape
+    dy, dskip = dy.contiguous(), dskip.contiguous()
+    dx = torch.empty_like(x)
+    rc = _L().rsuper_maxpool2_bwd_add(_DT[x.dtype], _ptr(x), C, _ptr(dy), C, _ptr(dskip), C, _ptr(dx), C, N, D, H, W, C, _stream())
+    if rc == 3:
+        return _maxpool_bwd(x, dy) + dskip
+    _l.check(rc, 'maxpool2_bwd_add')
+    return dx
+
+
 class MaxPoolFn(torch.autograd.Function):
 
     @staticmethod
     def forward(ctx, x):
-        _chk_act(x)
-        N, D, H, W, C = x.shape
-        OD, OH, OW = D // 2, H // 2, W // 2
-        y = torch.empty((N, OD, OH, OW, C), device=x.device, dtype=x.dtype)
-        blocks = _stat_blocks(OD * OH * OW)
-        part = torch.empty((N, blocks, C, 2), device=x.device, dtype=torch.float32)
-        _l.check(_L().rsuper_maxpool2_fwd(_DT[x.dtype], _ptr(x), C, _ptr(y), C, _ptr(part), blocks, N, D, H, W, C, _stream()), 'maxpool2_fwd')
-        mr = stats_finalize(part, OD * OH * OW)
+        y, mr = _maxpool_fwd(x)
         ctx.save_for_backward(x)
         ctx.mark_non_differentiable(mr)
         ctx.set_materialize_grads(False)
@@ -642,11 +676,7 @@
     @staticmethod
     def backward(ctx, dy, _unused):
         (x,) = ctx.saved_tensors
-        dy = dy.contiguous()
-        N, D, H, W, C = x.shape
-        dx = torch.empty_like(x)
-        _l.check(_L().rsuper_maxpool2_bwd(_DT[x.dtype], _ptr(x), C, _ptr(dy), C, _ptr(dx), C, N, D, H, W, C, _stream()), 'maxpool2_bwd')
-        return dx
+        return _maxpool_bwd(x, dy)
 
 
 _MaxPoolFn = MaxPoolFn
@@ -666,14 +696,54 @@
         if dskip is None:
             return _MaxPoolFn.backward(ctx, dy, None)
         (x,) = ctx.saved_tensors
+        return _maxpool_bwd_add(x, dy, dskip)
+
+
+def maxpool_lazy_plan(x):
+    N, D, H, W, C = x.shape
+    return x.dtype in _DT and _L().rsuper_maxpool2_bwd_lazy_plan(_DT[x.dtype], N, D, H, W, C) == 1
+
+
+def _rows(g):
+    N, D, H, W, C = g.shape
+    ld = g.stride(3)
+    if g.stride(4) == 1 and ld >= C and ld % 8 == 0 and g.stride() == (D * H * W * ld, H * W * ld, W * ld, ld, 1):
+        return g, ld
+    return g.contiguous(), C
+
+
+def _finalized(g, x, mr, gm):
+    if g is None or gm is None:
+        return g
+    return in_bwd_finalize(Src(g.contiguous()), Src(x, mr=mr), gm.contiguous(), g.shape[-1])
+
+
+class MaxPoolSkipLazyFn(torch.autograd.Function):
+
+    @staticmethod
+    def forward(ctx, x, mrx):
+        y, mr = _maxpool_fwd(x)
+        ctx.save_for_backward(x, mrx, y, mr)
+        ctx.set_materialize_grads(False)
+        return y, mr, x.view_as(x), mrx.view_as(mrx)
+
+    @staticmethod
+    def backward(ctx, dy, gmy, dskip, gmx):
+        x, mrx, y, mry = ctx.saved_tensors
         N, D, H, W, C = x.shape
-        dy, dskip = dy.contiguous(), dskip.contiguous()
-        dx = torch.empty_like(x)
-        rc = _L().rsuper_maxpool2_bwd_add(_DT[x.dtype], _ptr(x), C, _ptr(dy), C, _ptr(dskip), C, _ptr(dx), C, N, D, H, W, C, _stream())
-        if rc == 3:
-            return _MaxPoolFn.backward(ctx, dy, None) + dskip
-        _l.check(rc, 'maxpool2_bwd_add')
-        return dx
+        if dy is not None and dskip is not None and (gmy is not None or gmx is not None):
+            (dy, lddy), (dskip, lda) = _rows(dy), _rows(dskip)
+            gmy, gmx = (None if gmy is None else gmy.contiguous()), (None if gmx is None else gmx.contiguous())
+            dx = torch.empty_like(x)
+            rc = _L().rsuper_maxpool2_bwd_lazy(_DT[x.dtype], _ptr(x), C, _ptr(dy), lddy, _ptr(mry), _ptr(gmy), _ptr(dskip), lda, _ptr(mrx), _ptr(gmx),
+                                               _ptr(dx), C, N, D, H, W, C, _stream())
+            if rc != 3:
+                _l.check(rc, 'maxpool2_bwd_lazy')
+                return dx, None
+        dy, dskip = _finalized(dy, y, mry, gmy), _finalized(dskip, x, mrx, gmx)
+        if dy is None:
+            return dskip, None
+        return (_maxpool_bwd(x, dy) if dskip is None else _maxpool_bwd_add(x, dy, dskip)), None
 
 
 def subsample2(x, with_stats=True):
@@ -692,19 +762,32 @@
     _l.check(_L().rsuper_subsample2_bwd(_DT[dy.dtype], _ptr(dy), C, _ptr(out, off), out.shape[-1], N, D, H, W, C, _stream()), 'subsample2_bwd')
 
 
+def _upsample_fwd(x, size):
+    _chk_act(x)
+    N, ID, IH, IW, C = x.shape
+    OD, OH, OW = size
+    y = torch.empty((N, OD, OH, OW, C), device=x.device, dtype=x.dtype)
+    blocks = _stat_blocks(OD * OH * OW)
+    part = torch.empty((N, blocks, C, 2), device=x.device, dtype=torch.float32)
+    _l.check(_L().rsuper_upsample_fwd(_DT[x.dtype], _ptr(x), C, _ptr(y), C, _ptr(part), blocks, N, ID, IH, IW, OD, OH, OW, C, _stream()),
+              'upsample_fwd')
+    return y, stats_finalize(part, OD * OH * OW)
+
+
+def _upsample_bwd(in_shape, dy):
+    dy = dy.contiguous()
+    N, ID, IH, IW, C = in_shape
+    OD, OH, OW = dy.shape[1:4]
+    dx = torch.empty(in_shape, device=dy.device, dtype=dy.dtype)
+    _l.check(_L().rsuper_upsample_bwd(_DT[dy.dtype], _ptr(dy), C, _ptr(dx), C, N, ID, IH, IW, OD, OH, OW, C, _stream()), 'upsample_bwd')
+    return dx
+
+
 class UpsampleFn(torch.autograd.Function):
 
     @staticmethod
     def forward(ctx, x, size):
-        _chk_act(x)
-        N, ID, IH, IW, C = x.shape
-        OD, OH, OW = size
-        y = torch.empty((N, OD, OH, OW, C), device=x.device, dtype=x.dtype)
-        blocks = _stat_blocks(OD * OH * OW)
-        part = torch.empty((N, blocks, C, 2), device=x.device, dtype=torch.float32)
-        _l.check(_L().rsuper_upsample_fwd(_DT[x.dtype], _ptr(x), C, _ptr(y), C, _ptr(part), blocks, N, ID, IH, IW, OD, OH, OW, C, _stream()),
-                  'upsample_fwd')
-        mr = stats_finalize(part, OD * OH * OW)
+        y, mr = _upsample_fwd(x, size)
         ctx.in_shape = tuple(x.shape)
         ctx.mark_non_differentiable(mr)
         ctx.set_materialize_grads(False)
@@ -712,12 +795,40 @@
 
     @staticmethod
     def backward(ctx, dy, _unused):
-        dy = dy.contiguous()
-        N, ID, IH, IW, C = ctx.in_shape
-        OD, OH, OW = dy.shape[1:4]
-        dx = torch.empty(ctx.in_shape, device=dy.device, dtype=dy.dtype)
-        _l.check(_L().rsuper_upsample_bwd(_DT[dy.dtype], _ptr(dy), C, _ptr(dx), C, N, ID, IH, IW, OD, OH, OW, C, _stream()), 'upsample_bwd')
-        return dx, None
+        return _upsample_bwd(ctx.in_shape, dy), None
+
+
+def upsample_lazy_plan(x, size):
+    N, ID, IH, IW, C = x.shape
+    return x.dtype in _DT and _L().rsuper_upsample_bwd_lazy_plan(_DT[x.dtype], N, ID, IH, IW, *size, C) == 1
+
+
+class UpsampleLazyFn(torch.autograd.Function):
+
+    @staticmethod
+    def forward(ctx, x, size):
+        y, mr = _upsample_fwd(x, size)
+        ctx.in_shape = tuple(x.shape)
+        ctx.save_for_backward(y, mr)
+        ctx.set_materialize_grads(False)
+        return y, mr
+
+    @staticmethod
+    def backward(ctx, dy, gm):
+        if dy is None:
+            return None, None
+        u, mr = ctx.saved_tensors
+        if gm is not None:
+            N, ID, IH, IW, C = ctx.in_shape
+            OD, OH, OW = u.shape[1:4]
+            (g, ldg), gm = _rows(dy), gm.contiguous()
+            dx = torch.empty(ctx.in_shape, device=u.device, dtype=u.dtype)
+            rc = _L().rsuper_upsample_bwd_lazy(_DT[u.dtype], _ptr(g), ldg, _ptr(u), C, _ptr(mr), _ptr(gm), _ptr(dx), C,
+                                               N, ID, IH, IW, OD, OH, OW, C, _stream())
+            if rc != 3:
+                _l.check(rc, 'upsample_bwd_lazy')
+                return dx, None
+        return _upsample_bwd(ctx.in_shape, _finalized(dy, u, mr, gm)), None
 
 
 class StemFn(torch.autograd.Function):
diff --git a/r-super_amd/model/dim3/unet.py b/r-super_amd/model/dim3/unet.py
--- a/r-super_amd/model/dim3/unet.py
+++ b/r-super_amd/model/dim3/unet.py
@@ -51,13 +51,13 @@
         _lib.require_device()
         dt = self._dtype()
         x1, m1 = self.inc(x, dt)
-        x2, m2, x1 = self.down1(x1, m1, True)
-        x3, m3, x2 = self.down2(x2, m2, True)
-        x4, m4, x3 = self.down3(x3, m3, True)
-        x5, m5, x4 = self.down4(x4, m4, True)
-        o, mo = self.up1(x5, m5, x4, m4)
-        o, mo = self.up2(o, mo, x3, m3)
-        o, mo = self.up3(o, mo, x2, m2)
-        o, mo = self.up4(o, mo, x1, m1)
+        x2, m2, x1, s1 = self.down1(x1, m1, True, True)
+        x3, m3, x2, s2 = self.down2(x2, m2, True, True)
+        x4, m4, x3, s3 = self.down3(x3, m3, True, True)
+        x5, m5, x4, s4 = self.down4(x4, m4, True, True)
+        o, mo = self.up1(x5, m5, x4, s4)
+        o, mo = self.up2(o, mo, x3, s3)
+        o, mo = self.up3(o, mo, x2, s2)
+        o, mo = self.up4(o, mo, x1, s1)
         logits = ops.HeadFn.apply(o, self.outc.weight, self.outc.bias)
         return {'segmentation': logits}
diff --git a/r-super_amd/model/dim3/unet_utils.py b/r-super_amd/model/dim3/unet_utils.py
--- a/r-super_amd/model/dim3/unet_utils.py
+++ b/r-super_amd/model/dim3/unet_utils.py
@@ -7,7 +7,9 @@
 
 class _Pool(nn.Module):
 
-    def forward(self, x, with_skip=False):
+    def forward(self, x, with_skip=False, mr=None):
+        if mr is not None:
+            return ops.MaxPoolSkipLazyFn.apply(x, mr)
         return ops.MaxPoolSkipFn.apply(x) if with_skip else ops.MaxPoolFn.apply(x)
 
 
@@ -37,17 +39,22 @@
             layers.append(block(out_ch, out_ch, kernel_size=kernel_size, norm=norm))
         self.conv = nn.Sequential(*layers)
 
-    def forward(self, x, mr, with_skip=False):
+    def forward(self, x, mr, with_skip=False, lazy=False):
         blocks = list(self.conv)
-        skip = x
+        skip, mr_skip = x, mr
         if self.pool:
             if with_skip and torch.is_grad_enabled() and x.requires_grad:
-                x, mr, skip = blocks[0](x, True)
+                if lazy and ops.maxpool_lazy_plan(x):
+                    x, mr, skip, mr_skip = blocks[0](x, True, mr)
+                else:
+                    x, mr, skip = blocks[0](x, True)
             else:
                 x, mr = blocks[0](x)
             blocks = blocks[1:]
         for blk in blocks:
             x, mr = blk(x, mr)
+        if with_skip and lazy:
+            return x, mr, skip, mr_skip
         return (x, mr, skip) if with_skip else (x, mr)
 
 
@@ -60,7 +67,9 @@
         self.conv = nn.Sequential(*layers)
 
     def forward(self, x1, mr1, x2, mr2):
-        up, mru = ops.UpsampleFn.apply(x1, tuple(x2.shape[1:4]))
+        size = tuple(x2.shape[1:4])
+        lazy = torch.is_grad_enabled() and x1.requires_grad and ops.upsample_lazy_plan(x1, size)
+        up, mru = (ops.UpsampleLazyFn if lazy else ops.UpsampleFn).apply(x1, size)
         x, mr = self.conv[0](x2, mr2, up, mru)
         for blk in list(self.conv)[1:]:
             x, mr = blk(x, mr)
```

Result: faster. 176.0 million voxels/s, median of 6 (+1.0%).
